# KudanLimited/cuda-bundle-adjustment

Measured on AMD Instinct MI355X. Metric: ba_edge_iterations_per_sec, higher is better.
Workload: dtype f64

## Files before the change

### cuda-bundle-adjustment_amd/csrc/host/c_api.cpp

```cpp
#include <cmath>
#include <cstring>
#include <deque>
#include <memory>
#include <unordered_map>

#include "../../../include/cugo_hip.h"
#include "../../include/cuda_graph_optimisation.h"
#include "../../include/icp_types.h"
#include "../kernels/kernels.h"
#include "chol_solver.h"
#include "edge_layout.h"
#include "engine.h"
#include "hip_util.h"
#include "rccl_comm.h"
#include "schur_plan.h"

using namespace cugo_host;

namespace
{
template <typename F>
int guarded(F&& f)
{
    try
// ... 83 lines not shown
        CUGO_HIP(hipMemcpyAsync(d, h, bytes, hipMemcpyHostToDevice, ctx->stream));
        CUGO_HIP(hipStreamSynchronize(ctx->stream));
    });
}
int cugo_memcpy_d2h(cugo_ctx* ctx, void* h, const void* d, size_t bytes)
{
    return guarded([&] {
        CUGO_HIP(hipMemcpyAsync(h, d, bytes, hipMemcpyDeviceToHost, ctx->stream));
        CUGO_HIP(hipStreamSynchronize(ctx->stream));
    });
}
int cugo_memset(cugo_ctx* ctx, void* d, int value, size_t bytes)
{
    return guarded([&] { CUGO_HIP(hipMemsetAsync(d, value, bytes, ctx->stream)); });
}

int cugo_compute_active_errors(cugo_ctx* ctx, const cugo_edges* ev, const double* d_poses,
                               const double* d_lms, cugo_robust rk, double* d_chi)
{
    return guarded([&] {
        cugo_k::launch_errors(ctx->stream, *ev, d_poses, d_lms, rk, scratch_for(ctx, ev), d_chi);
        CUGO_HIP(hipGetLastError());
    });
}

int cugo_construct_quadratic_form(cugo_ctx* ctx, const cugo_edges* ev, const double* d_poses,
                                  const double* d_lms, cugo_robust rk, double* d_Hpp, double* d_bp,
                                  double* d_Hll, double* d_bl, void* d_Hpl, double* d_chi)
{
    return guarded([&] {
        cugo_k::launch_build(ctx->stream, *ev, d_poses, d_lms, rk, d_Hpp, d_bp, d_Hll, d_bl, d_Hpl,
                             scratch_for(ctx, ev), d_chi);
        CUGO_HIP(hipGetLastError());
    });
}

}

namespace
{
void check_icp_kind(cugo_ctx* ctx, const char* what, int n, int P, const int32_t* d_pose, const int32_t* d_ptr,
                    const double* d_p, const double* d_geo, const double* d_omega, int n_omega, int rk, double delta)
{
    const std::string in = std::string(" (") + what + ")";
    if (n < 0)
        throw std::runtime_error("cugo_icp: negative edge count" + in);
    if (!d_ptr)
        throw std::runtime_error("cugo_icp: no pose_ptr" + in);
    if (rk < CUGO_RK_NONE || rk > CUGO_RK_HUBER || (rk != CUGO_RK_NONE && !(delta > 0.0 && std::isfinite(delta))))
        throw std::runtime_error("cugo_icp: unknown robust kernel or bad delta" + in);
    if (n > 0 && (!d_pose || !d_p || !d_geo || !d_omega || (n_omega != 1 && n_omega != n)))
        throw std::runtime_error("cugo_icp: missing arrays" + in);
    std::vector<int32_t> ptr(P + 1);
    CUGO_HIP(hipMemcpyAsync(ptr.data(), d_ptr, sizeof(int32_t) * (P + 1), hipMemcpyDeviceToHost, ctx->stream));
    CUGO_HIP(hipStreamSynchronize(ctx->stream));
    if (ptr[0] != 0 || ptr[P] != n)
        throw std::runtime_error("cugo_icp: pose_ptr does not span the edges" + in);
    for (int p = 0; p < P; p++)
        if (ptr[p + 1] < ptr[p])
            throw std::runtime_error("cugo_icp: pose_ptr not ascending" + in);
}

void check_icp(cugo_ctx* ctx, const cugo_icp_edges* ev, cugo_k::ReduceScratch rs)
{
    check_icp_kind(ctx, "plane", ev->n_plane, ev->n_poses_total, ev->d_plane_pose, ev->d_plane_pose_ptr, ev->d_plane_p,
                   ev->d_plane_nd, ev->d_plane_omega, ev->n_plane_omega, ev->rk_plane, ev->delta_plane);
    check_icp_kind(ctx, "line", ev->n_line, ev->n_poses_total, ev->d_line_pose, ev->d_line_pose_ptr, ev->d_line_p,
                   ev->d_line_au, ev->d_line_omega, ev->n_line_omega, ev->rk_line, ev->delta_line);
    if (cugo_k::icp_check_indices(ctx->stream, *ev, rs))
        throw std::runtime_error("cugo_icp: edges not sorted by pose, or a pose index disagrees with pose_ptr");
}

void check_icp_counts(const cugo_icp_edges* ev)
{
    if (!ev || ev->n_poses_total < 0 || ev->n_poses_free < 0 || ev->n_poses_free > ev->n_poses_total ||
        ev->n_plane < 0 || ev->n_line < 0)
        throw std::runtime_error("cugo_icp: bad pose or edge counts");
}

cugo_k::ReduceScratch icp_scratch_for(cugo_ctx* ctx, const cugo_icp_edges* ev)
{
    const size_t need = cugo_k::icp_scratch_doubles(*ev);
    if (ctx->scratch.size() < need)
    {
        CUGO_HIP(hipStreamSynchronize(ctx->stream));
        ctx->scratch.resize(need);
    }
    return {ctx->scratch.data(), ctx->scratch.size()};
}
}

extern "C" {

int cugo_icp_compute_errors(cugo_ctx* ctx, const cugo_icp_edges* ev, const double* d_poses, double* d_chi,
                            double* d_edge_chi)
{
    return guarded([&] {
        check_icp_counts(ev);
        const cugo_k::ReduceScratch rs = icp_scratch_for(ctx, ev);
        check_icp(ctx, ev, rs);
        cugo_k::launch_icp_errors(ctx->stream, *ev, d_poses, rs, d_chi, false, d_edge_chi);
        CUGO_HIP(hipGetLastError());
    });
}

int cugo_icp_construct_quadratic_form(cugo_ctx* ctx, const cugo_icp_edges* ev, const double* d_poses, double* d_Hpp,
                                      double* d_bp, double* d_chi)
{
    return guarded([&] {
        check_icp_counts(ev);
        const cugo_k::ReduceScratch rs = icp_scratch_for(ctx, ev);
        check_icp(ctx, ev, rs);
        cugo_k::launch_icp_build(ctx->stream, *ev, d_poses, d_Hpp, d_bp, rs, d_chi, false);
        CUGO_HIP(hipGetLastError());
    });
}

int cugo_max_diagonal(cugo_ctx* ctx, const double* d_Hpp, int nP, const double* d_Hll, int nL,
                      double* d_out)
{
    return guarded([&] {
        cugo_k::launch_max_diagonal(ctx->stream, d_Hpp, nP, d_Hll, nL, scratch_for(ctx, nullptr),
                                    d_out);
        CUGO_HIP(hipGetLastError());
    });
}

int cugo_compute_schur(cugo_ctx* ctx, const cugo_edges* ev, const cugo_hsc_struct* hs, double lambda,
                       int damp_hsc_diag, const double* d_Hpp, const double* d_bp,
                       const double* d_Hll, const double* d_bl, const void* d_Hpl,
                       double* d_invHll, void* d_T, double* d_bsc, double* d_Hsc)
{
    return guarded([&] {
        if (!d_T && !hs->d_grp_ptr)
            throw std::runtime_error("cugo_compute_schur: d_T may only be NULL with a landmark-major plan "
                                     "(cugo_hsc_plan_create); the gather kernels read T from memory");
        cugo_k::SchurRows form;
        form.mfma = ctx->opt.hsc_mfma, form.xcd = ctx->opt.hsc_xcd;
        cugo_k::launch_schur(ctx->stream, *ev, *hs, lambda, damp_hsc_diag, d_Hpp, d_bp, d_Hll, d_bl,
                             d_Hpl, d_invHll, d_T, d_bsc, d_Hsc, false, form);
        CUGO_HIP(hipGetLastError());
    });
}

int cugo_backsubst_update(cugo_ctx* ctx, const cugo_edges* ev, double lambda,
                          const double* d_invHll, const double* d_bl, const double* d_bp,
                          const void* d_Hpl, const double* d_xp, double* d_xl,
                          const double* d_poses_in, const double* d_lms_in, double* d_poses_out,
                          double* d_lms_out, double* d_scale)
{
    return guarded([&] {
        cugo_k::launch_backsubst_update(ctx->stream, *ev, lambda, lambda, d_invHll, d_bl, d_bp, d_Hpl,
                                        d_xp, d_xl, d_poses_in, d_lms_in, d_poses_out, d_lms_out,
                                        scratch_for(ctx, ev), d_scale);
        CUGO_HIP(hipGetLastError());
    });
}

int cugo_chol_create(cugo_ctx* ctx, cugo_chol** out)
{
    return guarded([&] {
        auto* s = new cugo_chol;
        s->ctx = ctx;
        *out = s;
    });
}
void cugo_chol_destroy(cugo_chol* s)
{
    if (s && s->ctx)
        (void)hipStreamSynchronize(s->ctx->stream);
    delete s;
}
int cugo_chol_analyze(cugo_chol* s, int n, const int32_t* rowptr, const int32_t* colind)
{
    return guarded([&] { s->analyze(n, rowptr, colind); });
}
int cugo_chol_factor_solve(cugo_chol* s, const double* d_Hsc, double lambda, const double* d_bsc,
                           double* d_x, int32_t* d_fail)
{
    return guarded([&] {
        if (!s->analyzed || !s->ctx)
            throw std::runtime_error("cugo_chol_factor_solve needs an analysed solver with a device context");
        s->factor_solve(d_Hsc, lambda, d_bsc, d_x, d_fail);
    });
}
int cugo_chol_selected_inverse(cugo_chol* s, double* d_sigma)
{
    bool ok = true;
    const int rc = guarded([&] {
        if (!s || !s->ctx || !s->analyzed || !s->factored)
            throw std::runtime_error("cugo_chol_selected_inverse needs a factorisation (cugo_chol_factor_solve) since the "
                                     "last analyze()");
        if (s->own_subtrees())
            throw std::runtime_error("cugo_chol_selected_inverse: not available when the solver factors rank-owned "
                                     "subtrees");
        ok = s->selected_inverse(d_sigma);
    });
    if (rc != CUGO_OK)
        return rc;
    if (!ok)
    {
        set_last_error("cugo_chol_selected_inverse: the factorisation hit a zero pivot");
        return CUGO_ERR_NUMERIC;
    }
    return CUGO_OK;
}
#ifdef CUGO_DEBUG_HOOKS
int cugo_debug_pin_reference(void)
{
    return guarded([&] { cugo_debug_pin_reference_solver(); });
}
int cugo_debug_dump_call(int which, int call, const char* path)
{
    return guarded([&] {
        cugo_chol* s = cugo_debug_solver(which);
        if (!s)
            throw std::runtime_error("cugo_debug_dump_call: no solver has run with CUGO_DEBUG_KEEP");
        s->dump_slot(call, path);
    });
}
int cugo_debug_plan_array(int which, const char* name, const int32_t** out)
{
    cugo_chol* s = cugo_debug_solver(which);
    if (!s)
        return -1;
    return cugo_chol_plan_array(s, name, out);
}
int cugo_debug_dump(const char* dir, int* n_calls)
{
    return guarded([&] {
        const int n = cugo_debug_dump_last_solver(dir);
        if (n_calls)
            *n_calls = n;
    });
}
#endif
int cugo_chol_stats(const cugo_chol* s, double* nnzL, double* flops, int* n_super, int* n_stages,
                    double* front_bytes)
{
    if (nnzL)
        *nnzL = s->plan.nnzL;
    if (flops)
        *flops = s->plan.flops;
    if (n_super)
        *n_super = s->plan.n_super;
    if (n_stages)
        *n_stages = s->plan.n_stages;
    if (front_bytes)
        *front_bytes = 8.0 * (double)s->plan.front_doubles;
    return CUGO_OK;
}
int cugo_chol_plan_sizes(const cugo_chol* s, int* n, int* n_super, int* n_rows_total)
{
    *n = s->plan.n;
    *n_super = s->plan.n_super;
    *n_rows_total = (int)s->plan.rows.size();
    return CUGO_OK;
}
int cugo_chol_plan_get(const cugo_chol* s, int32_t* perm, int32_t* super_ptr, int32_t* rows_ptr,
                       int32_t* rows, int32_t* parent)
{
    const CholPlan& P = s->plan;
    std::memcpy(perm, P.perm.data(), sizeof(int32_t) * P.perm.size());
    std::memcpy(super_ptr, P.super_ptr.data(), sizeof(int32_t) * P.super_ptr.size());
    std::memcpy(rows_ptr, P.rows_ptr.data(), sizeof(int32_t) * P.rows_ptr.size());
    std::memcpy(rows, P.rows.data(), sizeof(int32_t) * P.rows.size());
    std::memcpy(parent, P.sparent.data(), sizeof(int32_t) * P.sparent.size());
    return CUGO_OK;
}

int cugo_chol_plan_array(cugo_chol* s, const char* name, const int32_t** out)
{
    const CholPlan& P = s->plan;
    const std::string n(name);
    const std::vector<int32_t>* v = nullptr;
#define CUGO_PLAN_FIELD(f) \
    if (n == #f)           \
    v = &P.f
    CUGO_PLAN_FIELD(perm);
    CUGO_PLAN_FIELD(super_ptr);
    CUGO_PLAN_FIELD(rows_ptr);
    CUGO_PLAN_FIELD(rows);
    CUGO_PLAN_FIELD(sparent);
    CUGO_PLAN_FIELD(child_ptr);
    CUGO_PLAN_FIELD(child);
    CUGO_PLAN_FIELD(rel_ptr);
    CUGO_PLAN_FIELD(rel);
    CUGO_PLAN_FIELD(ncb);
    CUGO_PLAN_FIELD(nb);
    CUGO_PLAN_FIELD(col0);
    CUGO_PLAN_FIELD(col_front);
    CUGO_PLAN_FIELD(stage_task_ptr);
    CUGO_PLAN_FIELD(task_ptr);
    CUGO_PLAN_FIELD(task_fronts);
    CUGO_PLAN_FIELD(blk_front);
    CUGO_PLAN_FIELD(blk_row);
    CUGO_PLAN_FIELD(blk_col);
    CUGO_PLAN_FIELD(alias_of);
    CUGO_PLAN_FIELD(asm_map);
    CUGO_PLAN_FIELD(wl);
    CUGO_PLAN_FIELD(bc_front);
    CUGO_PLAN_FIELD(bc_seg_ptr);
    CUGO_PLAN_FIELD(bc_seg);
#undef CUGO_PLAN_FIELD
    if (n == "asm_info")
    {
        s->asm_info.assign(1, P.asm0);
        s->asm_info.push_back(P.nasm);
        for (int64_t o : P.asm_off)
            s->asm_info.push_back((int32_t)o);
        v = &s->asm_info;
    }
    if (n == "blk_trans")
        v = &s->trans32;
    if (n == "ea1")
        v = &s->ea1;
    if (!v)
    {
        set_last_error("cugo_chol_plan_array: unknown array " + n);
        return CUGO_ERR_INVALID;
    }
    *out = v->data();
    return (int)v->size();
}

int cugo_chol_plan_array64(cugo_chol* s, const char* name, const int64_t** out)
{
    const CholPlan& P = s->plan;
    const std::string n(name);
    const std::vector<int64_t>* v = n == "off" ? &P.off : n == "ldf" ? &P.ldf : n == "woff" ? &P.woff
                                  : n == "l21off" ? &P.l21off : nullptr;
    if (!v)
    {
        set_last_error("cugo_chol_plan_array64: unknown array " + n);
        return CUGO_ERR_INVALID;
    }
    *out = v->data();
    return (int)v->size();
}

int cugo_shard_range(int n_landmarks_total, const int32_t* edges_per_landmark, int rank, int world,
                     int* l0, int* l1)
{
    return guarded([&] {
        if (world < 1 || rank < 0 || rank >= world)
            throw std::runtime_error("cugo_shard_range: bad rank/world");
        std::vector<int32_t> cnt(n_landmarks_total + 1, 0);
        for (int l = 0; l < n_landmarks_total; l++)
            cnt[l + 1] = cnt[l] + edges_per_landmark[l];
        shard_range(cnt, rank, world, *l0, *l1);
    });
}

struct cugo_graph
{
    cugo::GraphOptimisationOptions options;
    std::unique_ptr<cugo::CudaGraphOptimisationImpl> opt;
    cugo::PoseVertexSet poses{false};
    cugo::LandmarkVertexSet lms{true};
    cugo::MonoEdgeSet mono;
    cugo::StereoEdgeSet stereo;
    cugo::PlaneEdgeSet plane;
    cugo::LineEdgeSet line;
    std::deque<cugo::PlaneEdge> plane_store;
    std::deque<cugo::LineEdge> line_store;
    std::deque<cugo::PoseVertex> pose_store;
    std::deque<cugo::LandmarkVertex> lm_store;
    std::deque<cugo::MonoEdge> mono_store;
    std::deque<cugo::StereoEdge> stereo_store;
    bool attached = false;
    void attach()
    {
        if (attached)
            return;
        opt->addVertexSet(&poses);
        opt->addVertexSet(&lms);
        opt->addEdgeSet(&mono);
        opt->addEdgeSet(&stereo);
        opt->addEdgeSet(&plane);
        opt->addEdgeSet(&line);
        attached = true;
    }
};

int cugo_graph_create(int per_edge_information, int per_edge_camera, cugo_graph** out)
{
    return guarded([&] {
        auto g = std::make_unique<cugo_graph>();
        g->options.perEdgeInformation = per_edge_information != 0;
        g->options.perEdgeCamera = per_edge_camera != 0;
        g->opt = std::make_unique<cugo::CudaGraphOptimisationImpl>(g->options);
        *out = g.release();
    });
}
struct cugo_hsc_plan
{
    cugo_host::SchurPlanDevice dev;
};
int cugo_hsc_plan_create(cugo_ctx* ctx, int n_edges, int n_poses_free, const int32_t* h_pose, const int32_t* h_lm,
                         const uint8_t* h_flags, const int32_t* h_rowptr, const int32_t* h_colind,
                         cugo_hsc_struct* hs, cugo_hsc_plan** out)
{
    int rc = guarded([&] {
        if (!ctx || !hs || !out)
            throw std::runtime_error("cugo_hsc_plan_create: null argument");
        *out = nullptr;
        cugo_host::SchurPlanDevice::clear(*hs);
        cugo_host::SchurPlanHost h;
        cugo_host::build_schur_plan(n_edges, n_poses_free, h_pose, h_lm, h_flags, h_rowptr, h_colind, h);
        if (!h.usable)
            throw std::invalid_argument("cugo_hsc_plan_create: a landmark's active edges straddle two 256-slot groups");
        auto p = std::make_unique<cugo_hsc_plan>();
        p->dev.upload(h, ctx->stream);
        p->dev.fill(*hs);
        *out = p.release();
    });
    return rc;
}
void cugo_hsc_plan_destroy(cugo_hsc_plan* plan) { delete plan; }

int cugo_graph_create_plan_only(int per_edge_information, int per_edge_camera, cugo_graph** out)
{
    return guarded([&] {
        auto g = std::make_unique<cugo_graph>();
        g->options.perEdgeInformation = per_edge_information != 0;
        g->options.perEdgeCamera = per_edge_camera != 0;
        g->options.planOnly = true;
        g->opt = std::make_unique<cugo::CudaGraphOptimisationImpl>(g->options);
        *out = g.release();
    });
}
void cugo_graph_destroy(cugo_graph* g) { delete g; }

int cugo_graph_add_poses(cugo_graph* g, int n, const int32_t* ids, const double* qt, const uint8_t* fixed)
{
    return guarded([&] {
        for (int i = 0; i < n; i++)
        {
            g->pose_store.emplace_back(ids[i], cugo::Se3D(qt + 7 * (size_t)i, qt + 7 * (size_t)i + 4),
                                       fixed && fixed[i]);
            g->poses.addVertex(&g->pose_store.back());
        }
    });
}
int cugo_graph_add_landmarks(cugo_graph* g, int n, const int32_t* ids, const double* xyz,
                             const uint8_t* fixed)
{
    return guarded([&] {
        for (int i = 0; i < n; i++)
        {
            g->lm_store.emplace_back(ids[i], cugo::Vec3d(xyz + 3 * (size_t)i), fixed && fixed[i]);
            g->lms.addVertex(&g->lm_store.back());
        }
    });
}
int cugo_graph_add_edges(cugo_graph* g, int dim, int n, const int32_t* pose_ids, const int32_t* lm_ids,
                         const double* meas, const double* info, const double* cam5)
{
    return guarded([&] {
        if (dim != 2 && dim != 3)
            throw std::runtime_error("cugo_graph_add_edges: dim must be 2 or 3");
        for (int i = 0; i < n; i++)
        {
            cugo::PoseVertex* vp = g->poses.getVertex(pose_ids[i]);
            cugo::LandmarkVertex* vl = g->lms.getVertex(lm_ids[i]);
            cugo::Camera cam;
            if (cam5)
                cam = cugo::Camera(cam5[5 * (size_t)i], cam5[5 * (size_t)i + 1], cam5[5 * (size_t)i + 2],
                                   cam5[5 * (size_t)i + 3], cam5[5 * (size_t)i + 4]);
            if (dim == 2)
            {
                g->mono_store.emplace_back();
                cugo::MonoEdge& e = g->mono_store.back();
                e.setVertex(vp, 0), e.setVertex(vl, 1);
                e.setMeasurement(cugo::Vec2d(meas + 2 * (size_t)i));
                e.setInformation(info ? info[i] : 0.0);
                if (cam5)
                    e.setCamera(cam);
                g->mono.addEdge(&e);
            }
            else
            {
                g->stereo_store.emplace_back();
                cugo::StereoEdge& e = g->stereo_store.back();
                e.setVertex(vp, 0), e.setVertex(vl, 1);
                e.setMeasurement(cugo::Vec3d(meas + 3 * (size_t)i));
                e.setInformation(info ? info[i] : 0.0);
                if (cam5)
                    e.setCamera(cam);
                g->stereo.addEdge(&e);
            }
        }
    });
}
static cugo::PoseVertex* icp_pose(cugo_graph* g, int32_t id)
{
    try
    {
        return g->poses.getVertex(id);
    }
    catch (const std::out_of_range&)
    {
        throw std::invalid_argument("cugo_graph_add_*_edges: unknown pose id " + std::to_string(id));
    }
}
int cugo_graph_add_plane_edges(cugo_graph* g, int n, const int32_t* pose_ids, const double* pointP,
                               const double* normal, const double* origin_distance, const double* info)
{
    return guarded([&] {
        if (n < 0 || (n > 0 && (!pose_ids || !pointP || !normal || !origin_distance)))
            throw std::invalid_argument("cugo_graph_add_plane_edges: missing arrays");
        for (int i = 0; i < n; i++)
            (void)icp_pose(g, pose_ids[i]);
        for (int i = 0; i < n; i++)
        {
            g->plane_store.emplace_back();
            cugo::PlaneEdge& e = g->plane_store.back();
            e.setVertex(icp_pose(g, pose_ids[i]), 0);
            e.setMeasurement(cugo::PointToPlaneMatch<double>(cugo::Vec3d(normal + 3 * (size_t)i), origin_distance[i],
                                                             cugo::Vec3d(pointP + 3 * (size_t)i)));
            e.setInformation(info ? info[i] : 0.0);
            g->plane.addEdge(&e);
        }
    });
}
int cugo_graph_add_line_edges(cugo_graph* g, int n, const int32_t* pose_ids, const double* pointP, const double* a,
                              const double* b, const double* info)
{
    return guarded([&] {
        if (n < 0 || (n > 0 && (!pose_ids || !pointP || !a || !b)))
            throw std::invalid_argument("cugo_graph_add_line_edges: missing arrays");
        for (int i = 0; i < n; i++)
            (void)icp_pose(g, pose_ids[i]);
        for (int i = 0; i < n; i++)
        {
            g->line_store.emplace_back();
            cugo::LineEdge& e = g->line_store.back();
            e.setVertex(icp_pose(g, pose_ids[i]), 0);
            cugo::PointToLineMatch<double> mz(cugo::Vec3d(a + 3 * (size_t)i), cugo::Vec3d(b + 3 * (size_t)i));
            mz.pointP = cugo::Vec3d(pointP + 3 * (size_t)i);
            e.setMeasurement(mz);
            e.setInformation(info ? info[i] : 0.0);
            g->line.addEdge(&e);
        }
    });
}
static cugo::BaseEdgeSet* icp_set(cugo_graph* g, int kind)
{
    if (kind == CUGO_ICP_PLANE)
        return &g->plane;
    if (kind == CUGO_ICP_LINE)
        return &g->line;
    throw std::invalid_argument("cugo: kind must be CUGO_ICP_PLANE (0) or CUGO_ICP_LINE (1)");
}
int cugo_graph_set_icp_information(cugo_graph* g, int kind, double info)
{
    return guarded([&] { icp_set(g, kind)->setInformation(info); });
}
int cugo_graph_set_icp_robust_kernel(cugo_graph* g, int kind, int type, double delta)
{
    return guarded([&] {
        const cugo::RobustKernelType t = type == CUGO_RK_CAUCHY  ? cugo::RobustKernelType::Cauchy
                                         : type == CUGO_RK_TUKEY ? cugo::RobustKernelType::Tukey
                                         : type == CUGO_RK_HUBER ? cugo::RobustKernelType::Huber
                                                                 : cugo::RobustKernelType::None;
        icp_set(g, kind)->setRobustKernel(t, delta);
    });
}
int cugo_graph_set_icp_outlier_threshold(cugo_graph* g, int kind, double threshold)
{
    return guarded([&] {
        if (kind == CUGO_ICP_PLANE)
            g->plane.setOutlierThreshold(threshold);
        else if (kind == CUGO_ICP_LINE)
            g->line.setOutlierThreshold(threshold);
        else
            icp_set(g, kind);
    });
}
int cugo_graph_n_icp_edges(cugo_graph* g, int kind)
{
    return kind == CUGO_ICP_PLANE || kind == CUGO_ICP_LINE ? g->opt->nIcpEdges(kind) : -1;
}
int cugo_graph_set_camera(cugo_graph* g, int dim, const double* c)
{
    const cugo::Camera cam(c[0], c[1], c[2], c[3], c[4]);
    if (dim == 3)
        g->stereo.setCamera(cam);
    else
        g->mono.setCamera(cam);
    return CUGO_OK;
}
int cugo_graph_set_information(cugo_graph* g, int dim, double info)
{
    if (dim == 3)
        g->stereo.setInformation(info);
    else
        g->mono.setInformation(info);
    return CUGO_OK;
}
int cugo_graph_set_robust_kernel(cugo_graph* g, int dim, int type, double delta)
{
    const cugo::RobustKernelType t = type == CUGO_RK_CAUCHY  ? cugo::RobustKernelType::Cauchy
                                     : type == CUGO_RK_TUKEY ? cugo::RobustKernelType::Tukey
                                     : type == CUGO_RK_HUBER ? cugo::RobustKernelType::Huber
                                                             : cugo::RobustKernelType::None;
// ... 282 lines not shown
```

### cuda-bundle-adjustment_amd/csrc/host/chol_solver.cpp

```cpp
#include "chol_solver.h"

#include <cstdio>
#include <cstdlib>
#include <cstring>
#include <string>

using namespace cugo_host;

void cugo_chol::pack()
{
    const CholPlan& P = plan;
    pack32.clear(), pack64.clear();
    auto put32 = [this](const std::vector<int32_t>& v) {
        const size_t o = pack32.size();
        pack32.insert(pack32.end(), v.begin(), v.end());
        pack32.resize((pack32.size() + 3) & ~size_t(3));
        return o;
    };
    auto put64 = [this](const std::vector<int64_t>& v) {
        const size_t o = pack64.size();
        pack64.insert(pack64.end(), v.begin(), v.end());
        pack64.resize((pack64.size() + 1) & ~size_t(1));
        return o;
    };
    const size_t o_ncb = put32(P.ncb), o_nb = put32(P.nb), o_col0 = put32(P.col0);
    const size_t o_alias = put32(P.alias_of), o_bwnp = put32(P.bw_np), o_lanp = put32(P.la_np);
    const size_t o_rows_ptr = put32(P.rows_ptr), o_rows = put32(P.rows);
    const size_t o_child_ptr = put32(P.child_ptr), o_child = put32(P.child);
    const size_t o_rel_ptr = put32(P.rel_ptr), o_rel = put32(P.rel);
    const size_t o_task_ptr = put32(P.task_ptr), o_task_fronts = put32(P.task_fronts);
    const size_t o_blk_front = put32(P.blk_front), o_blk_row = put32(P.blk_row), o_blk_col = put32(P.blk_col);
    const size_t o_perm = put32(P.perm), o_col_front = put32(P.col_front), o_wl = put32(P.wl);
    const size_t ntask = P.task_ptr.empty() ? 0 : P.task_ptr.size() - 1;
    constexpr int R = cugo_k::EA1_REC;
    std::vector<int32_t> ea1_ptr(P.n_super + 1, 0);
    ea1.clear();
    for (int f = 0; f < P.n_super; f++)
    {
        if (P.alias_of[f] < 0)
            for (int k = P.child_ptr[f]; k < P.child_ptr[f + 1]; k++)
            {
                const int c = P.child[k];
                const int64_t ncs_c = 6 * (int64_t)P.ncb[c], ldc = P.ldf[c];
                const int64_t q[2] = {P.off[c] + ncs_c * ldc + ncs_c, ldc};
                int32_t r[R] = {c, P.nb[c] - P.ncb[c], P.la_np[c], P.rel_ptr[c]};
                std::memcpy(r + 4, q, sizeof q);
                uint32_t mask = 0;
                for (int b = 0; b < P.la_np[c]; b++)
                {
                    const int pr = P.rel[P.rel_ptr[c] + b];
                    if (pr < 0 || pr >= 32 || pr >= P.ncb[f])
                        throw std::runtime_error("cugo: a child's leading row lies outside its parent's pivot block");
                    mask |= 1u << pr;
                }
                r[8] = (int32_t)mask;
                ea1.insert(ea1.end(), r, r + R);
            }
        ea1_ptr[f + 1] = (int32_t)(ea1.size() / R);
    }
    const size_t n_ea1 = ea1.size();
    ea1.resize(n_ea1 + R, 0);
    const size_t o_ea1 = put32(ea1);
    ea1.resize(n_ea1);
    std::vector<int32_t> tmeta(cugo_k::TMETA * ntask, 0);
    for (size_t t = 0; t < ntask; t++)
    {
        int32_t* m = tmeta.data() + cugo_k::TMETA * t;
        const int f = P.task_fronts[P.task_ptr[t]];
        m[0] = P.task_ptr[t + 1] - P.task_ptr[t], m[1] = f, m[2] = P.ncb[f], m[3] = P.nb[f], m[4] = P.col0[f];
        m[5] = P.bw_np[f], m[6] = P.rows_ptr[f];
        m[7] = (P.alias_of[f] < 0 && P.child_ptr[f + 1] > P.child_ptr[f]) ? 1 : 0;
        m[16] = ea1_ptr[f], m[17] = ea1_ptr[f + 1];
        for (int q = 0; q < 16; q++)
        {
            const int nrows = P.rows_ptr[f + 1] - P.rows_ptr[f];
            m[20 + q] = nrows > 0 ? P.rows[P.rows_ptr[f] + std::min(q, nrows - 1)] : 0;
        }
        const int64_t q[4] = {P.off[f], P.ldf[f], P.woff[f], P.l21off[f]};
        std::memcpy(m + 8, q, sizeof q);
    }
    const size_t o_tmeta = put32(tmeta);
    std::vector<int32_t> fat(16 * (P.wl.size() / 3), 0);
    for (size_t i = 0; i < P.wl.size() / 3; i++)
    {
        int32_t* m = fat.data() + 16 * i;
        const int f = P.wl[3 * i];
        m[0] = f, m[1] = P.wl[3 * i + 1], m[2] = P.wl[3 * i + 2];
        if (f < 0 || f >= P.n_super)
            continue;
        m[3] = 6 * P.ncb[f], m[4] = 6 * (P.nb[f] - P.ncb[f]);
        m[5] = P.bw_np[f], m[6] = P.col0[f], m[7] = P.rows_ptr[f];
        const int64_t q[4] = {P.off[f], P.ldf[f], P.woff[f], P.l21off[f]};
        std::memcpy(m + 8, q, sizeof q);
        if ((int)i >= P.asm0 && (int)i < P.asm0 + P.nasm)
        {
            const int64_t nb = P.nb[f], mo = P.asm_off[f];
            m[5] = (int32_t)nb;
            std::memcpy(m + 6, &mo, sizeof mo);
            bool any = false;
            for (int64_t cb = m[1]; cb < m[2]; cb++)
            {
                any = any || P.asm_map[mo + cb] >= 0;
                const int64_t c0 = mo + nb + cb * nb - cb * (cb - 1) / 2;
                for (int64_t k = 0; k < nb - cb && !any; k++)
                    any = P.asm_map[c0 + k] >= 0;
            }
            m[4] = any ? 1 : 0;
        }
    }
    const size_t o_fat = put32(fat);
    std::vector<int32_t> bc_rec(cugo_k::BC_REC * P.bc_front.size(), 0), bc_seg(4 * (P.bc_seg.size() / 3) + 4, 0);
    for (size_t t = 0; t < P.bc_front.size(); t++)
    {
        int32_t* m = bc_rec.data() + cugo_k::BC_REC * t;
        const int f = P.bc_front[t];
        m[0] = f, m[1] = P.ncb[f], m[2] = P.nb[f], m[3] = P.col0[f], m[4] = P.rows_ptr[f];
        m[5] = P.bc_seg_ptr[f], m[6] = P.bc_seg_ptr[f + 1] - P.bc_seg_ptr[f];
        const int64_t q[4] = {P.woff[f], P.l21off[f], P.off[f], P.ldf[f]};
        std::memcpy(m + 8, q, sizeof q);
    }
    for (size_t k = 0; k < P.bc_seg.size() / 3; k++)
        std::memcpy(bc_seg.data() + 4 * k, P.bc_seg.data() + 3 * k, 3 * sizeof(int32_t));
    const size_t o_bc_rec = put32(bc_rec), o_bc_seg = put32(bc_seg);
    const size_t o_asm_map = put32(P.asm_map);
    const size_t o_trans = pack32.size();
    pack32.resize(o_trans + (P.blk_trans.size() + 3) / 4 + 4, 0);
    if (!P.blk_trans.empty())
        std::memcpy(pack32.data() + o_trans, P.blk_trans.data(), P.blk_trans.size());
    const size_t o_asm_off = put64(P.asm_off);
    const size_t o_off = put64(P.off), o_woff = put64(P.woff), o_l21off = put64(P.l21off), o_ldf = put64(P.ldf);
    po = {o_ncb, o_nb, o_col0, o_alias, o_bwnp, o_lanp, o_rows_ptr, o_rows, o_child_ptr, o_child, o_rel_ptr, o_rel,
          o_task_ptr, o_task_fronts, o_blk_front, o_blk_row, o_blk_col, o_perm, o_col_front, o_wl, o_ea1, o_tmeta,
          o_fat, o_asm_map, o_trans, o_asm_off, o_off, o_woff, o_l21off, o_ldf, o_bc_rec, o_bc_seg};
}

void cugo_chol::upload(hipStream_t s)
{
    const CholPlan& P = plan;
    const size_t o_ncb = po[0], o_nb = po[1], o_col0 = po[2], o_alias = po[3], o_bwnp = po[4], o_lanp = po[5];
    const size_t o_rows_ptr = po[6], o_rows = po[7], o_child_ptr = po[8], o_child = po[9], o_rel_ptr = po[10];
    const size_t o_rel = po[11], o_task_ptr = po[12], o_task_fronts = po[13], o_blk_front = po[14], o_blk_row = po[15];
    const size_t o_blk_col = po[16], o_perm = po[17], o_col_front = po[18], o_wl = po[19], o_ea1 = po[20];
    const size_t o_tmeta = po[21], o_fat = po[22], o_asm_map = po[23], o_trans = po[24], o_asm_off = po[25];
    const size_t o_off = po[26], o_woff = po[27], o_l21off = po[28], o_ldf = po[29];
    const size_t o_bc_rec = po[30], o_bc_seg = po[31];
    d_pack32.upload(pack32, s), d_pack64.upload(pack64, s);
    d_fronts.resize((size_t)P.front_doubles + 16);
    d_fronts.zero(s);
    d_xnew.resize((size_t)6 * P.n + 16);
    d_junk.resize(64 * 1024);
    d_winv.resize((size_t)P.winv_doubles + 16);
    d_l21.resize((size_t)P.l21_doubles + 16);
    bw_chain = opt.bw_chain && !opt.lookahead && !P.has_subtree_stage && !P.bc_front.empty();
    if (bw_chain)
    {
        d_bc_state.resize((size_t)cugo_k::BC_DONE + P.n_super);
        d_bc_state.zero(s);
        h_bc_error.resize(1);
        h_bc_error[0] = 0;
        bc_base = 0, bc_epoch = 0;
    }
    CUGO_HIP(hipStreamSynchronize(s));

    cugo_k::CholPlanDev& D = dev;
    D.n_fronts = P.n_super;
    const int32_t* b32 = d_pack32.data();
    const int64_t* b64 = d_pack64.data();
    D.ncb = b32 + o_ncb, D.nb = b32 + o_nb, D.off = b64 + o_off, D.col0 = b32 + o_col0;
    D.rows_ptr = b32 + o_rows_ptr, D.rows = b32 + o_rows;
    D.child_ptr = b32 + o_child_ptr, D.child = b32 + o_child;
    D.rel_ptr = b32 + o_rel_ptr, D.rel = b32 + o_rel;
    D.n_stages = P.n_stages;
    D.task_ptr = b32 + o_task_ptr, D.task_fronts = b32 + o_task_fronts, D.tmeta = b32 + o_tmeta;
    D.n_hsc_blocks = (int)P.blk_front.size();
    D.blk_front = b32 + o_blk_front, D.blk_row = b32 + o_blk_row;
    D.blk_col = b32 + o_blk_col, D.blk_trans = reinterpret_cast<const uint8_t*>(b32 + o_trans);
    D.n = P.n, D.perm = b32 + o_perm, D.col_front = b32 + o_col_front;
    D.junk = d_junk.data();
    D.woff = b64 + o_woff, D.winv = d_winv.data(), D.nc_max = P.nc_max;
    D.ea_lds = opt.ea_lds, D.panel16 = opt.panel16, D.ea_direct = opt.ea_direct;
#ifdef CUGO_DEBUG_HOOKS
    {
        const char* ka = std::getenv("CUGO_KERNEL_ACQUIRE");
        D.kernel_acquire = ka ? std::atoi(ka) & 7 : 0;
        const char* ed = std::getenv("CUGO_DEBUG_DELAY");
        D.dbg_delay = ed ? std::atoi(ed) : 0;
        const char* ez = std::getenv("CUGO_DEBUG_ZERO_LDS");
        D.zero_lds = ez ? std::atoi(ez) : 0, D.lds_doubles = 0;
        D.dbg_skip_wg = -1;
    }
#endif
    D.l21off = b64 + o_l21off, D.l21 = d_l21.data();
    D.ldf = b64 + o_ldf, D.alias_of = b32 + o_alias, D.bw_np = b32 + o_bwnp, D.la_np = b32 + o_lanp;
    d_wl_ptr = b32 + o_wl;
    D.wl_base = d_wl_ptr, D.fat = b32 + o_fat, D.ea1 = b32 + o_ea1;
    D.asm_map = b32 + o_asm_map, D.asm_off = b64 + o_asm_off;
    D.bc_rec = b32 + o_bc_rec, D.bc_seg = b32 + o_bc_seg;
    asm_fronts = opt.asm_fronts;
    lds_factor = cugo_k::chol_lds_factor_bytes(P.nc_max);
    lds_backward = cugo_k::chol_lds_backward_bytes(P.nc_max, P.ld_max);
}

void cugo_chol::analyze(int n, const int32_t* rowptr, const int32_t* colind)
{
    analyze_host(n, rowptr, colind);
    if (ctx)
        upload(ctx->stream);
}

void cugo_chol::analyze_host(int n, const int32_t* rowptr, const int32_t* colind)
{
    CholOptions copt = CholOptions::from_env();
    const bool own_forced = opt.own_subtrees == 1;
    if ((world > 1 || own_forced) && bcast && opt.own_subtrees != 0)
        copt.rank = rank, copt.world = world, copt.owned = true;
    chol_analyze(n, rowptr, colind, copt, plan);
    if (copt.owned && !own_forced && plan.flops < 1e9 * opt.own_min_gflop)
    {
        copt.rank = 0, copt.world = 1, copt.owned = false;
        chol_analyze(n, rowptr, colind, copt, plan);
    }
    lookahead = opt.lookahead;
    factored = false, si_ready = false, last_fail = nullptr;
    trans32.assign(plan.blk_trans.begin(), plan.blk_trans.end());
    pack();
    if (plan.nc_max > cugo_k::chol_max_pivot_cols() ||
        cugo_k::chol_lds_factor_bytes(plan.nc_max) > 160 * 1024 ||
        cugo_k::chol_lds_backward_bytes(plan.nc_max, plan.ld_max) > 160 * 1024)
        throw std::runtime_error("cugo: a front exceeds the LDS budget (nc=" +
                                 std::to_string(plan.nc_max) + ", ld=" + std::to_string(plan.ld_max) + ")");
    analyzed = true;
}

#ifdef CUGO_DEBUG_HOOKS
static cugo_chol* g_last_kept = nullptr;
static cugo_chol* g_ref_kept = nullptr;
cugo_chol::~cugo_chol()
{
    if (g_last_kept == this)
        g_last_kept = nullptr;
    if (g_ref_kept == this)
        g_ref_kept = nullptr;
}
void cugo_chol::dump_kept(const char* dir)
{
    CUGO_HIP(hipStreamSynchronize(ctx->stream));
    const size_t nf = (size_t)plan.front_doubles, nw = (size_t)plan.winv_doubles, nl = (size_t)plan.l21_doubles,
                 nx = (size_t)6 * plan.n;
    for (size_t c = 0; c < keep.size(); c++)
    {
        std::vector<double> h(nf + nw + nl + 2 * nx);
        if (keep[c]->size() < h.size())
            continue;
        CUGO_HIP(hipMemcpy(h.data(), keep[c]->data(), h.size() * sizeof(double), hipMemcpyDeviceToHost));
        const std::string path = std::string(dir) + "/call" + std::to_string(c) + ".bin";
        std::FILE* f = std::fopen(path.c_str(), "wb");
        if (!f)
            throw std::runtime_error("cugo_debug_dump: cannot write " + path);
        const int64_t hdr[8] = {(int64_t)nf, (int64_t)nw, (int64_t)nl, (int64_t)nx, (int64_t)nx, 0, 0, 0};
        std::fwrite(hdr, sizeof hdr, 1, f);
        std::fwrite(h.data(), sizeof(double), h.size(), f);
        std::fclose(f);
    }
}
int cugo_debug_dump_last_solver(const char* dir)
{
    if (!g_last_kept)
        return 0;
    g_last_kept->dump_kept(dir);
    return (int)g_last_kept->keep.size();
}
cugo_chol* cugo_debug_solver(int which) { return which ? g_ref_kept : g_last_kept; }
void cugo_debug_pin_reference_solver() { g_ref_kept = g_last_kept; }
void cugo_chol::dump_slot(int call, const char* path)
{
    CUGO_HIP(hipStreamSynchronize(ctx->stream));
    const size_t nf = (size_t)plan.front_doubles, nw = (size_t)plan.winv_doubles, nl = (size_t)plan.l21_doubles,
                 nx = (size_t)6 * plan.n, total = nf + nw + nl + 2 * nx;
    if (call < 0 || call >= (int)keep.size() || keep[call]->size() < total)
        throw std::runtime_error("cugo_debug_dump_call: no such slot");
    std::vector<double> h(total);
    CUGO_HIP(hipMemcpy(h.data(), keep[call]->data(), total * sizeof(double), hipMemcpyDeviceToHost));
    std::FILE* f = std::fopen(path, "wb");
    if (!f)
        throw std::runtime_error(std::string("cugo_debug_dump_call: cannot write ") + path);
    const int64_t hdr[8] = {(int64_t)nf, (int64_t)nw, (int64_t)nl, (int64_t)nx, (int64_t)nx, 0, 0, 0};
    std::fwrite(hdr, sizeof hdr, 1, f);
    std::fwrite(h.data(), sizeof(double), h.size(), f);
    std::fclose(f);
}

struct cugo_chol_hooks
{
    cugo_chol& c;
    hipStream_t s;
    bool skip_on = false;
    double* stale_line = nullptr;
    int stale_stage = -1, stale_kind = -1;
    bool hash_levels, gap, keep_on;
    explicit cugo_chol_hooks(cugo_chol& solver) : c(solver), s(solver.ctx->stream)
    {
        const char* hl = std::getenv("CUGO_DEBUG_HASH_LEVELS");
        hash_levels = !(hl && hl[0] == '0');
        gap = std::getenv("CUGO_DEBUG_GAP") != nullptr;
        keep_on = std::getenv("CUGO_DEBUG_KEEP") != nullptr;
        const cugo_host::CholPlan& plan = c.plan;
        const char* sk = std::getenv("CUGO_DEBUG_SKIP");
        const char* dump = c.dbg_calls == 0 ? std::getenv("CUGO_DEBUG_SKIP_DUMP") : nullptr;
        int cc = -1, l = -1, w = -1;
        if (sk && std::sscanf(sk, "%d:%d:%d", &cc, &l, &w) == 3 && cc == c.dbg_calls)
            cugo_k::chol_dbg_skip_begin(l, w, dump), skip_on = true;
        else if (dump)
            cugo_k::chol_dbg_skip_begin(-1, -1, dump), skip_on = true;
        c.dbg_calls++;
        const char* sl = std::getenv("CUGO_DEBUG_STALE");
        int kind = -1;
        long line = -1;
        if (sl && std::sscanf(sl, "%d:%d:%ld", &cc, &kind, &line) == 3 && cc == c.dbg_calls - 1 && line >= 0)
        {
            std::vector<int> stage_of(plan.n_super, 0);
            for (int st = 0; st < plan.n_stages; st++)
                for (int t = plan.stage_task_ptr[st]; t < plan.stage_task_ptr[st + 1]; t++)
                    for (int fi = plan.task_ptr[t]; fi < plan.task_ptr[t + 1]; fi++)
                        stage_of[plan.task_fronts[fi]] = st;
            const int64_t e = 16 * (int64_t)line;
            if (kind == 0 && e + 16 <= plan.winv_doubles)
            {
                int f = 0;
                for (int k = 0; k < plan.n_super; k++)
                    if (plan.woff[k] <= e && plan.woff[k] >= plan.woff[f])
                        f = k;
                stale_line = c.d_winv.data() + e, stale_stage = stage_of[f], stale_kind = 0;
            }
            else if (kind == 1 && e + 16 <= 6LL * plan.n)
                stale_line = c.d_xnew.data() + e, stale_stage = stage_of[plan.col_front[e / 6]], stale_kind = 1;
            if (stale_line)
            {
                c.dbg_scratch.resize(16);
                CUGO_HIP(hipMemcpyAsync(c.dbg_scratch.data(), stale_line, 16 * sizeof(double), hipMemcpyDeviceToDevice, s));
            }
        }
    }
    ~cugo_chol_hooks()
    {
        if (skip_on)
            cugo_k::chol_dbg_skip_end();
    }
    void hash(int slot, const double* ptr, size_t n)
    {
        if (c.dbg_hash && slot < 64)
            cugo_k::launch_hash_words(s, ptr, n, c.dbg_hash + slot);
    }
    void after_level(int st)
    {
        if (hash_levels && st < 24)
        {
            hash(16 + st, c.d_winv.data(), (size_t)c.plan.winv_doubles);
            hash(40 + st, c.d_fronts.data(), (size_t)c.plan.front_doubles);
        }
        if (gap)
            cugo_k::launch_nop(s);
    }
    double* stale_for_potrf(int st) const { return stale_kind == 0 && stale_stage == st ? stale_line : nullptr; }
    void after_two_phase(int st)
    {
        if (stale_kind == 0 && stale_stage == st)
            cugo_k::launch_swap16(s, stale_line, c.dbg_scratch.data());
    }
    void after_backward(int st)
    {
        if (stale_kind == 1 && (st == stale_stage || st == stale_stage - 1))
            cugo_k::launch_swap16(s, stale_line, c.dbg_scratch.data());
    }
    void keep_arrays(double* d_x)
    {
        if (!keep_on || c.dbg_calls > 16)
            return;
        const cugo_host::CholPlan& plan = c.plan;
        const size_t nf = (size_t)plan.front_doubles, nw = (size_t)plan.winv_doubles, nl = (size_t)plan.l21_doubles,
                     nx = (size_t)6 * plan.n;
        while (c.keep.size() < (size_t)c.dbg_calls)
            c.keep.emplace_back(new cugo_host::DevBuf<double>());
        auto& k = *c.keep[c.dbg_calls - 1];
        k.resize(nf + nw + nl + 2 * nx + 8);
        double* dst = k.data();
        const std::pair<const double*, size_t> parts[] = {{c.d_fronts.data(), nf}, {c.d_winv.data(), nw}, {c.d_l21.data(), nl},
                                                          {c.d_xnew.data(), nx}, {d_x, nx}};
        for (const auto& pr : parts)
        {
            if (pr.second)
                CUGO_HIP(hipMemcpyAsync(dst, pr.first, pr.second * sizeof(double), hipMemcpyDeviceToDevice, s));
            dst += pr.second;
        }
        g_last_kept = &c;
    }
};
#define CUGO_HOOK(expr) expr
#else
cugo_chol::~cugo_chol() {}
#define CUGO_HOOK(expr) ((void)0)
#endif

void cugo_chol::factor_solve(const double* d_Hsc, double lambda, const double* d_bsc, double* d_x,
                             int32_t* d_fail)
{
    hipStream_t s = ctx->stream;
    check_chain_error();
    factored = true, last_fail = d_fail;
#ifdef CUGO_DEBUG_HOOKS
    cugo_chol_hooks hooks(*this);
#endif
#ifdef CUGO_STAMPS
    static const bool dbg = std::getenv("CUGO_DEBUG_STAMPS") != nullptr;
    static long long* d_stamps = nullptr;
    if (dbg && !d_stamps)
    {
        CUGO_HIP(hipMalloc(reinterpret_cast<void**>(&d_stamps), 64 * sizeof(long long)));
        CUGO_HIP(hipMemset(d_stamps, 0, 64 * sizeof(long long)));
        cugo_k::set_debug_stamps(d_stamps);
    }
#endif
    cugo_k::launch_chol_assemble(s, dev, d_fronts.data(), (size_t)plan.front_doubles, d_Hsc, lambda, d_bsc, d_fail,
                                 d_wl_ptr + 3L * plan.clr0, plan.nclr, asm_fronts ? d_wl_ptr + 3L * plan.asm0 : nullptr,
                                 plan.nasm);
    CUGO_HOOK(hooks.hash(11, d_fronts.data(), (size_t)plan.front_doubles));
    int pend0 = 0, npend = 0, pend_tile = 64;
    for (int st = 0; st < plan.n_stages; st++)
    {
        const int t0 = plan.stage_task_ptr[st], t1 = plan.stage_task_ptr[st + 1];
        if (plan.has_subtree_stage && st == 0)
            cugo_k::launch_chol_subtree_stage(s, dev, d_fronts.data(), t0, t1 - t0, lds_factor, d_fail);
        else if (lookahead)
        {
            cugo_k::launch_chol_potrf_la(s, dev, d_fronts.data(), t0, t1 - t0, d_wl_ptr + 3L * pend0, npend,
                                         pend_tile, d_fail);
            cugo_k::launch_chol_lead(s, dev, d_fronts.data(), d_wl_ptr + 3L * plan.lead_ptr[st],
                                     plan.lead_ptr[st + 1] - plan.lead_ptr[st], d_wl_ptr + 3L * plan.ea_ptr[st],
                                     plan.ea_ptr[st + 1] - plan.ea_ptr[st], d_wl_ptr + 3L * plan.eab_ptr[st],
                                     plan.eab_ptr[st + 1] - plan.eab_ptr[st]);
            pend0 = plan.sb_ptr[st], npend = plan.sb_ptr[st + 1] - plan.sb_ptr[st];
            pend_tile = plan.stage_tile[st] ? plan.stage_tile[st] : 64;
        }
        else
        {
            double* stale = nullptr;
            double* stale_scratch = nullptr;
            CUGO_HOOK((stale = hooks.stale_for_potrf(st), stale_scratch = dbg_scratch.data()));
            cugo_k::launch_chol_upper_stage(
                s, dev, d_fronts.data(), t0, t1 - t0, d_wl_ptr, plan.ea_ptr[st],
                plan.ea_ptr[st + 1] - plan.ea_ptr[st], plan.eab_ptr[st],
                plan.eab_ptr[st + 1] - plan.eab_ptr[st], plan.syrk_ptr[st],
                plan.syrk_ptr[st + 1] - plan.syrk_ptr[st], plan.stage_tile[st], lds_factor, d_fail, stale, stale_scratch);
            if (plan.stage_tile[st] == 0)
            {
                cugo_k::launch_chol_two_phase(s, dev, d_fronts.data(), d_wl_ptr + 3L * plan.trsm_ptr[st],
                                              plan.trsm_ptr[st + 1] - plan.trsm_ptr[st],
                                              d_wl_ptr + 3L * plan.syrk_ptr[st],
                                              plan.syrk_ptr[st + 1] - plan.syrk_ptr[st]);
                CUGO_HOOK(hooks.after_two_phase(st));
            }
        }
        CUGO_HOOK(hooks.after_level(st));
        bool grouped = false;
        for (size_t k = 0; k < plan.xu_front.size(); k++)
            if (plan.xu_stage[k] == st)
            {
                if (!grouped && bcast_group)
                    bcast_group(true), grouped = true;
                const int f = plan.xu_front[k];
                const int64_t ld = plan.ldf[f], c0 = 6LL * plan.ncb[f], c1 = 6LL * plan.nb[f];
                if (c1 > c0)
                    bcast(d_fronts.data() + plan.off[f] + c0 * ld + c0, (size_t)((c1 - 1 - c0) * ld + c1 + 1 - c0),
                          plan.xu_owner[k]);
            }
        if (grouped)
            bcast_group(false);
    }
    if (npend > 0)
        cugo_k::launch_chol_potrf_la(s, dev, d_fronts.data(), 0, 0, d_wl_ptr + 3L * pend0, npend, pend_tile, d_fail);
    CUGO_HOOK(hooks.hash(12, d_winv.data(), (size_t)plan.winv_doubles));
    CUGO_HOOK(hooks.hash(13, d_l21.data(), (size_t)plan.l21_doubles));
    CUGO_HOOK(hooks.hash(14, d_fronts.data(), (size_t)plan.front_doubles));
    if (bw_chain)
    {
        const int nf = (int)plan.bc_front.size();
        if (++bc_epoch == 0)
            bc_epoch = 1;
        cugo_k::launch_chol_backward_chain(s, dev, d_fronts.data(), nf, d_xnew.data(), d_x, d_bc_state.data(), bc_base,
                                           bc_epoch, d_fail, h_bc_error.data());
        bc_base += (uint32_t)nf;
#ifdef CUGO_STAMPS
        if (dbg)
        {
            static int chain_calls = 0;
            static long long* d_cs = nullptr;
            if (++chain_calls == 4)
            {
                CUGO_HIP(hipMalloc(reinterpret_cast<void**>(&d_cs), 3 * sizeof(long long) * (size_t)nf));
                CUGO_HIP(hipMemset(d_cs, 0, 3 * sizeof(long long) * (size_t)nf));
                cugo_k::set_chain_stamps(d_cs);
            }
            if (chain_calls == 5)
            {
                std::vector<long long> h(3 * (size_t)nf);
                std::vector<int> ticket(plan.n_super, -1);
                for (int t = 0; t < nf; t++)
                    ticket[plan.bc_front[t]] = t;
                CUGO_HIP(hipStreamSynchronize(s));
                CUGO_HIP(hipMemcpy(h.data(), d_cs, h.size() * sizeof(long long), hipMemcpyDeviceToHost));
                cugo_k::set_chain_stamps(nullptr);
                long long first = h[0], last = 0;
                for (int t = 0; t < nf; t++)
                    first = std::min(first, h[3 * t]), last = std::max(last, h[3 * t + 2]);
                std::printf("chain stamps: %d fronts, first start to last done %lld ticks (10 ns)\n", nf, last - first);
                for (int f = plan.bc_front[nf - 1]; f >= 0; f = plan.sparent[f])
                {
                    const int t = ticket[f], pa = plan.sparent[f];
                    std::printf("  front %d ticket %d ncb %d rows %d: start +%lld", f, t, plan.ncb[f], plan.nb[f] - plan.ncb[f],
                                h[3 * t] - first);
                    if (pa >= 0)
                        std::printf(" wait %lld work %lld", h[3 * t + 1] - h[3 * ticket[pa] + 2], h[3 * t + 2] - h[3 * t + 1]);
                    std::printf(" done +%lld\n", h[3 * t + 2] - first);
                }
            }
        }
#endif
    }
    for (int st = plan.n_stages - 1; st >= 0 && !bw_chain; st--)
    {
        const int t0 = plan.stage_task_ptr[st], t1 = plan.stage_task_ptr[st + 1];
        cugo_k::launch_chol_backward_stage(s, dev, d_fronts.data(), t0, t1 - t0, lds_backward, d_xnew.data(),
                                           d_x, d_wl_ptr + 3L * plan.bwg_ptr[st],
                                           plan.bwg_ptr[st + 1] - plan.bwg_ptr[st]);
        CUGO_HOOK(hooks.after_backward(st));
#ifdef CUGO_STAMPS
        if (dbg && st == plan.n_stages - 1)
        {
            CUGO_HIP(hipStreamSynchronize(s));
            CUGO_HIP(hipMemcpy(d_stamps + 48, d_stamps + 24, 8 * sizeof(long long), hipMemcpyDeviceToDevice));
        }
#endif
    }
    CUGO_HOOK(hooks.hash(15, d_xnew.data(), (size_t)6 * plan.n));
    if (!plan.xx_lo.empty())
    {
        if (bcast_group)
            bcast_group(true);
        for (size_t k = 0; k < plan.xx_lo.size(); k++)
            bcast(d_xnew.data() + 6LL * plan.xx_lo[k], (size_t)(6LL * (plan.xx_hi[k] - plan.xx_lo[k])), plan.xx_owner[k]);
        if (bcast_group)
            bcast_group(false);
        cugo_k::launch_chol_unpermute(s, dev, d_xnew.data(), d_x);
    }
    CUGO_HIP(hipGetLastError());
    CUGO_HOOK(hooks.keep_arrays(d_x));
#ifdef CUGO_STAMPS
    if (dbg)
    {
        long long h[64];
        CUGO_HIP(hipStreamSynchronize(s));
        CUGO_HIP(hipMemcpy(h, d_stamps, sizeof h, hipMemcpyDeviceToHost));
        static int calls = 0;
        if (++calls == 5)
            for (int k = 0; k < 7; k++)
            {
                std::printf("stamps kernel %d (nc=%lld):", k, h[k * 8 + 6]);
                for (int i = 1; i < 8; i++)
                    if (i != 6 && h[k * 8 + i])
                        std::printf(" [%d] +%lld", i, h[k * 8 + i] - h[k * 8]);
                std::printf("  (cycles since kernel start; last launch of the kernel)\n");
            }
    }
#endif
}

void cugo_chol::check_chain_error()
{
    if (bw_chain && h_bc_error.data() && *static_cast<volatile uint32_t*>(h_bc_error.data()) != 0)
        throw std::runtime_error("cugo: the backward substitution gave up waiting for a front (k_backward_chain)");
}

bool cugo_chol::selected_inverse(double* d_sigma)
{
    hipStream_t s = ctx->stream;
    int32_t h_fail = 0;
    CUGO_HIP(hipMemcpyAsync(&h_fail, last_fail, sizeof h_fail, hipMemcpyDeviceToHost, s));
    CUGO_HIP(hipStreamSynchronize(s));
    check_chain_error();
    if (h_fail)
        return false;
    const CholPlan& P = plan;
    if (!si_ready)
    {
        std::vector<int64_t> sinfo(4 * (size_t)P.n_super + 4, 0);
        for (int f = 0; f < P.n_super; f++)
        {
            const int pa = P.sparent[f];
            if (pa < 0)
                continue;
            sinfo[4 * f] = P.off[pa], sinfo[4 * f + 1] = P.ldf[pa], sinfo[4 * f + 2] = P.rel_ptr[f];
            sinfo[4 * f + 3] = P.alias_of[pa] == f ? 0 : 1;
        }
        const int tile = cugo_k::selinv_row_tile();
        std::vector<int32_t> items;
        si_ptr.assign(P.n_stages + 1, 0);
        for (int st = 0; st < P.n_stages; st++)
        {
            si_ptr[st] = (int32_t)(items.size() / 2);
            if (!(P.has_subtree_stage && st == 0))
                for (int t = P.stage_task_ptr[st]; t < P.stage_task_ptr[st + 1]; t++)
                    for (int fi = P.task_ptr[t]; fi < P.task_ptr[t + 1]; fi++)
                    {
                        const int f = P.task_fronts[fi];
                        for (int r0 = 0; r0 < 6 * (P.nb[f] - P.ncb[f]); r0 += tile)
                            items.push_back(f), items.push_back(r0);
                    }
        }
        si_ptr[P.n_stages] = (int32_t)(items.size() / 2);
        items.resize(items.size() + 2, 0);
        d_sinfo.upload(sinfo, s);
        d_sitems.upload(items, s);
        d_sig.resize((size_t)P.front_doubles + 16);
        d_sig.zero(s);
        CUGO_HIP(hipStreamSynchronize(s));
        si_ready = true;
    }
    for (int st = P.n_stages - 1; st >= 0; st--)
    {
        const int t0 = P.stage_task_ptr[st], t1 = P.stage_task_ptr[st + 1];
        if (P.has_subtree_stage && st == 0)
            cugo_k::launch_selinv_subtree(s, dev, d_fronts.data(), d_sig.data(), d_sinfo.data(), t0, t1 - t0);
        else
        {
            cugo_k::launch_selinv_rows(s, dev, d_fronts.data(), d_sig.data(), d_sinfo.data(),
                                       d_sitems.data() + 2L * si_ptr[st], si_ptr[st + 1] - si_ptr[st]);
            cugo_k::launch_selinv_jj(s, dev, d_fronts.data(), d_sig.data(), t0, t1 - t0);
        }
    }
    cugo_k::launch_selinv_gather(s, dev, d_sig.data(), d_sigma);
    CUGO_HIP(hipGetLastError());
    return true;
}
```

### cuda-bundle-adjustment_amd/csrc/host/chol_solver.h

```cpp
#pragma once
#include "../kernels/kernels.h"
#include "chol_symbolic.h"
#include "hip_util.h"
#include "options.h"

#include <array>
#include <functional>
#include <memory>

struct cugo_chol
{
    cugo_ctx* ctx = nullptr;
    bool analyzed = false;
    cugo_host::Options opt = cugo_host::Options::from_env();
    cugo_host::CholPlan plan;
    std::vector<int32_t> trans32;
    std::vector<int32_t> asm_info;
    std::vector<int32_t> ea1;
    cugo_k::CholPlanDev dev{};
    size_t lds_factor = 0, lds_backward = 0;
    bool lookahead = false;
    bool asm_fronts = true;

    std::vector<int32_t> pack32;
    std::vector<int64_t> pack64;
    std::array<size_t, 32> po{};
    cugo_host::DevBuf<int32_t> d_pack32;
    cugo_host::DevBuf<int64_t> d_pack64;
    const int32_t* d_wl_ptr = nullptr;
    cugo_host::DevBuf<double> d_fronts, d_xnew, d_junk, d_winv, d_l21;
    bool bw_chain = false;
    cugo_host::DevBuf<uint32_t> d_bc_state;
    cugo_host::PinnedBuf<uint32_t> h_bc_error;
    uint32_t bc_base = 0, bc_epoch = 0;
    void check_chain_error();

    int rank = 0, world = 1;
    std::function<void(double*, size_t, int)> bcast;
    std::function<void(bool)> bcast_group;
    ~cugo_chol();
#ifdef CUGO_DEBUG_HOOKS
    unsigned long long* dbg_hash = nullptr;
    int dbg_calls = 0;
    std::vector<std::unique_ptr<cugo_host::DevBuf<double>>> keep;
    cugo_host::DevBuf<double> dbg_scratch;
    void dump_kept(const char* dir);
    void dump_slot(int call, const char* path);
#endif
    bool own_subtrees() const { return bcast && plan.owned; }

    const int32_t* last_fail = nullptr;
    bool factored = false;
    bool si_ready = false;
    cugo_host::DevBuf<double> d_sig;
    cugo_host::DevBuf<int64_t> d_sinfo;
    cugo_host::DevBuf<int32_t> d_sitems;
    std::vector<int32_t> si_ptr;
    bool selected_inverse(double* d_sigma);

    void analyze(int n, const int32_t* rowptr, const int32_t* colind);
    void analyze_host(int n, const int32_t* rowptr, const int32_t* colind);
    void pack();
    void upload(hipStream_t s);
    void factor_solve(const double* d_Hsc, double lambda, const double* d_bsc, double* d_x,
                      int32_t* d_fail);
};

#ifdef CUGO_DEBUG_HOOKS
int cugo_debug_dump_last_solver(const char* dir);
cugo_chol* cugo_debug_solver(int which);
void cugo_debug_pin_reference_solver();
#endif
```

### cuda-bundle-adjustment_amd/csrc/host/chol_symbolic.cpp

```cpp
#include "chol_symbolic.h"

#include <algorithm>
#include <atomic>
#include <chrono>
#include <cstdio>
#include <cstdlib>
#include <functional>
#include <numeric>
#include <stdexcept>
#include <thread>
#include <tuple>

namespace cugo_host
{

CholOptions CholOptions::from_env()
{
    CholOptions o;
    if (const char* s = std::getenv("CUGO_ND_LEAF"))
        o.nd_leaf = std::max(1, std::atoi(s));
    if (const char* s = std::getenv("CUGO_MAX_SUPER_COLS"))
        o.max_super_cols = std::max(1, std::atoi(s));
    if (const char* s = std::getenv("CUGO_ZERO_FRAC"))
        o.zero_frac = std::atof(s);
// ... 1176 lines not shown
        P.nc_max = std::max(P.nc_max, 6 * P.ncb[s]);
    P.ea_ptr.assign(1, 0), P.eab_ptr.assign(1, 0), P.syrk_ptr.assign(1, 0), P.bwg_ptr.assign(1, 0);
    P.lead_ptr.assign(1, 0), P.sb_ptr.assign(1, 0);
    P.bw_np.assign(ns, -1);
    P.la_np.assign(ns, 0);
    for (int c = 0; c < ns; c++)
        if (P.sparent[c] >= 0)
        {
            const int nbr = P.nb[c] - P.ncb[c], ncbp = P.ncb[P.sparent[c]];
            int np = 0;
            while (np < nbr && P.rel[P.rel_ptr[c] + np] < ncbp)
                np++;
            P.la_np[c] = np;
        }
    std::vector<int32_t> lead, sb;
    P.l21off.assign(ns, -1);
    P.l21_doubles = 0;
    std::vector<int32_t> ea, eab, sy, bwg, tr;
    std::vector<int> sy_front_ntiles;
    P.trsm_ptr.assign(1, 0);
    P.stage_tile.assign(P.n_stages, 64);
    for (int st = 0; st < P.n_stages; st++)
    {
        const bool subtree = P.has_subtree_stage && st == 0;
        int TS = 64;
        bool two_phase = false;
        if (!subtree)
        {
            long n64 = 0;
            for (int t = P.stage_task_ptr[st]; t < P.stage_task_ptr[st + 1]; t++)
            {
                const int f = P.task_fronts[P.task_ptr[t]];
                const long nti = (6 * (P.nb[f] - P.ncb[f]) + 1 + 63) / 64;
                n64 += nti * (nti + 1) / 2;
            }
            if (n64 <= opt.tile32_max_tiles)
                TS = 32;
            P.stage_tile[st] = TS;
            two_phase = opt.two_phase_min_tiles > 0 && n64 > opt.two_phase_min_tiles;
            if (two_phase)
                P.stage_tile[st] = 0;
        }
        if (!subtree)
            for (int t = P.stage_task_ptr[st]; t < P.stage_task_ptr[st + 1]; t++)
            {
                const int f = P.task_fronts[P.task_ptr[t]];
                const int nb = P.nb[f], ncb = P.ncb[f];
                {
                    const double nc = 6.0 * ncb, nr = 6.0 * (nb - ncb);
                    P.up_potrf_flops += nc * nc * nc / 3.0;
                    P.up_trsm_flops += nc * nc * (nr + 1);
                    P.up_syrk_flops += 2.0 * nc * (nr * (nr + 1) / 2 + nr);
                    for (int k = P.child_ptr[f]; k < P.child_ptr[f + 1] && P.alias_of[f] < 0; k++)
                    {
                        const double cr = 6.0 * (P.nb[P.child[k]] - P.ncb[P.child[k]]);
                        P.up_ea_bytes += 24.0 * (cr * (cr + 1) / 2 + cr);
                    }
                }
                if (P.child_ptr[f + 1] > P.child_ptr[f] && P.alias_of[f] < 0)
                {
                    const int chunks = (6 * nb + 1 + 63) / 64;
                    const int cols = std::max(1, std::min(8, 16 / chunks));
                    for (int c0 = 0; c0 < ncb; c0 += cols)
                    {
                        ea.push_back(f), ea.push_back(c0), ea.push_back(std::min(ncb, c0 + cols));
                    }
                    for (int c0 = ncb; c0 < nb; c0 += cols)
                    {
                        eab.push_back(f), eab.push_back(c0), eab.push_back(std::min(nb, c0 + cols));
                    }
                }
                const int nrs = 6 * (nb - ncb), nbelow = nrs + 1;
                const int nti = (nbelow + TS - 1) / TS, ntj = (nrs + TS - 1) / TS;
                const size_t sy_front0 = sy.size();
                if (two_phase)
                {
                    int ntl = 0;
                    for (int tj = 0; tj < ntj; tj++)
                        ntl += nti - tj;
                    for (int t = 0; t < ntl; t++)
                    {
                        sy.push_back(f), sy.push_back(t), sy.push_back(ntj);
                    }
                    for (int r0 = 0; r0 < nbelow; r0 += 64)
                    {
                        tr.push_back(f), tr.push_back(r0), tr.push_back(std::min(64, nbelow - r0));
                    }
                }
                else
                {
                    for (int tj = 0; tj < ntj; tj++)
                        for (int ti = tj; ti < nti; ti++)
                        {
                            sy.push_back(f), sy.push_back(ti), sy.push_back(tj);
                        }
                    for (int ti = ntj; ti < nti; ti++)
                    {
                        sy.push_back(f), sy.push_back(ti), sy.push_back(-1);
                    }
                }
                sy_front_ntiles.push_back(std::max(1, (int)((sy.size() - sy_front0) / 3)));
                const int q = 6 * P.la_np[f];
                if (q > 0)
                {
                    lead.push_back(f), lead.push_back(0), lead.push_back(0);
                }
                for (int tj = 0; tj < ntj; tj++)
                    for (int ti = tj; ti < nti; ti++)
                        if (TS * (ti + 1) > q)
                        {
                            sb.push_back(f), sb.push_back(ti), sb.push_back(tj);
                        }
                for (int ti = ntj; ti < nti; ti++)
                {
                    sb.push_back(f), sb.push_back(ti), sb.push_back(-1);
                }
                P.l21off[f] = P.l21_doubles;
                P.l21_doubles += (int64_t)6 * ncb * nbelow;
                for (int k = P.child_ptr[f]; k < P.child_ptr[f + 1]; k++)
                {
                    const int c = P.child[k];
                    if (lower[c] || !mine(c))
                        continue;
                    const int nbr = P.nb[c] - P.ncb[c];
                    int npb = 0;
                    while (npb < nbr && P.rel[P.rel_ptr[c] + npb] < ncb)
                        npb++;
                    if (nbr - npb >= 8)
                    {
                        P.bw_np[c] = npb;
                        for (int j0 = 0; j0 < 6 * P.ncb[c]; j0 += 16)
                        {
                            bwg.push_back(c), bwg.push_back(j0), bwg.push_back(0);
                        }
                    }
                }
            }
        if (!subtree && opt.xcd_affinity && !sy_front_ntiles.empty())
        {
            const int nf = (int)sy_front_ntiles.size();
            int total = 0;
            for (int n : sy_front_ntiles)
                total += n;
            if (total > 8)
            {
                std::vector<int> byn(nf);
                for (int i = 0; i < nf; i++)
                    byn[i] = i;
                std::stable_sort(byn.begin(), byn.end(), [&](int a, int b) { return sy_front_ntiles[a] > sy_front_ntiles[b]; });
                std::vector<int> load(8, 0);
                std::vector<int> group_of(P.n_super, 0);
                for (int i : byn)
                {
                    const int g = (int)(std::min_element(load.begin(), load.end()) - load.begin());
                    group_of[P.task_fronts[P.task_ptr[P.stage_task_ptr[st] + i]]] = g;
                    load[g] += sy_front_ntiles[i];
                }
                auto interleave = [&](std::vector<int32_t>& list, size_t first, int phase) {
                    const int n = (int)(list.size() / 3 - first);
                    if (n <= 1)
                        return;
                    std::vector<std::vector<int>> grp(8);
                    for (int k = 0; k < n; k++)
                        grp[group_of[list[3 * (first + k)]]].push_back(k);
                    std::vector<int32_t> out;
                    out.reserve((size_t)n * 3);
                    std::vector<size_t> pos(8, 0);
                    for (int k = 0; k < n; k++)
                    {
                        const int g = (phase + k) & 7;
                        int t;
                        if (pos[g] < grp[g].size())
                            t = grp[g][pos[g]++];
                        else
                        {
                            int best = 0;
                            size_t left = 0;
                            for (int h = 0; h < 8; h++)
                                if (grp[h].size() - pos[h] > left)
                                    left = grp[h].size() - pos[h], best = h;
                            t = grp[best].back();
                            grp[best].pop_back();
                        }
                        out.insert(out.end(), list.begin() + 3 * (first + t), list.begin() + 3 * (first + t) + 3);
                    }
                    std::copy(out.begin(), out.end(), list.begin() + 3 * first);
                };
                interleave(sy, (size_t)P.syrk_ptr.back(), 0);
                interleave(tr, (size_t)P.trsm_ptr.back(), 0);
            }
        }
        sy_front_ntiles.clear();
        P.ea_ptr.push_back((int)ea.size() / 3);
        P.eab_ptr.push_back((int)eab.size() / 3);
        P.syrk_ptr.push_back((int)sy.size() / 3);
        P.trsm_ptr.push_back((int)tr.size() / 3);
        P.bwg_ptr.push_back((int)bwg.size() / 3);
        P.lead_ptr.push_back((int)lead.size() / 3);
        P.sb_ptr.push_back((int)sb.size() / 3);
    }
    P.wl.clear();
    P.wl.insert(P.wl.end(), ea.begin(), ea.end());
    P.wl.insert(P.wl.end(), eab.begin(), eab.end());
    P.wl.insert(P.wl.end(), sy.begin(), sy.end());
    P.wl.insert(P.wl.end(), bwg.begin(), bwg.end());
    for (auto& v : P.eab_ptr)
        v += (int)ea.size() / 3;
    for (auto& v : P.syrk_ptr)
        v += (int)(ea.size() + eab.size()) / 3;
    for (auto& v : P.bwg_ptr)
        v += (int)(ea.size() + eab.size() + sy.size()) / 3;
    for (auto& v : P.trsm_ptr)
        v += (int)P.wl.size() / 3;
    P.wl.insert(P.wl.end(), tr.begin(), tr.end());
    P.clr0 = (int)P.wl.size() / 3;
    P.nclr = 0;
    for (int f = 0; f < ns; f++)
        if (P.alias_of[f] < 0 && mine(f))
            for (int c0 = 0; c0 < 6 * P.nb[f]; c0 += 16)
            {
                P.wl.push_back(f), P.wl.push_back(c0), P.wl.push_back(std::min(6 * P.nb[f], c0 + 16));
                P.nclr++;
            }
    P.asm0 = (int)P.wl.size() / 3;
    P.nasm = 0;
    P.asm_off.assign(ns, -1);
    P.asm_map.clear();
    {
        std::vector<int32_t> root(ns), shift(ns);
        for (int f = 0; f < ns; f++)
        {
            int o = f;
            while (P.alias_of[o] >= 0)
                o = P.alias_of[o];
            const int64_t delta = P.off[f] - P.off[o], ld = P.ldf[o];
            if (P.ldf[f] != ld || delta % (ld + 1) != 0 || (delta / (ld + 1)) % 6 != 0 ||
                delta / (ld + 1) / 6 + P.nb[f] != P.nb[o])
                throw std::runtime_error("cugo: a front stored inside another one is not on its diagonal");
            root[f] = o, shift[f] = (int)(delta / (ld + 1) / 6);
        }
        for (int f = 0; f < ns; f++)
            if (P.alias_of[f] < 0 && mine(f))
            {
                const int64_t nb = P.nb[f];
                P.asm_off[f] = (int64_t)P.asm_map.size();
                P.asm_map.resize(P.asm_map.size() + nb + nb * (nb + 1) / 2, -1);
                for (int cb = 0; cb < nb; cb += 2)
                {
                    P.wl.push_back(f), P.wl.push_back(cb), P.wl.push_back((int)std::min<int64_t>(nb, cb + 2));
                    P.nasm++;
                }
            }
        for (int f = 0; f < ns; f++)
            if (P.asm_off[root[f]] >= 0)
                for (int c = 0; c < P.ncb[f]; c++)
                    P.asm_map[P.asm_off[root[f]] + shift[f] + c] = P.col0[f] + c;
        for (size_t k = 0; k < P.blk_front.size(); k++)
        {
            const int f = P.blk_front[k], o = root[f];
            if (P.asm_off[o] < 0)
                continue;
            const int64_t nb = P.nb[o], rb = P.blk_row[k] + shift[f], cb = P.blk_col[k] + shift[f];
            if (rb < cb || rb >= nb)
                throw std::runtime_error("cugo: an Hsc block outside the lower triangle of its front");
            int32_t& e = P.asm_map[P.asm_off[o] + nb + cb * nb - cb * (cb - 1) / 2 + (rb - cb)];
            if (e != -1)
                throw std::runtime_error("cugo: two Hsc blocks in one front position");
            e = 2 * (int32_t)k + (rb != cb && P.blk_trans[k] ? 1 : 0);
        }
    }
    for (auto& v : P.lead_ptr)
        v += (int)P.wl.size() / 3;
    P.wl.insert(P.wl.end(), lead.begin(), lead.end());
    for (auto& v : P.sb_ptr)
        v += (int)P.wl.size() / 3;
    P.wl.insert(P.wl.end(), sb.begin(), sb.end());
    lap("8 work items");
    P.bc_front.clear(), P.bc_seg.clear();
    P.bc_seg_ptr.assign(ns + 1, 0);
    std::vector<int32_t> ticket(ns, -1);
    for (int st = P.n_stages - 1; st >= 0; st--)
        for (int t = P.stage_task_ptr[st]; t < P.stage_task_ptr[st + 1]; t++)
            for (int fi = P.task_ptr[t + 1] - 1; fi >= P.task_ptr[t]; fi--)
            {
                ticket[P.task_fronts[fi]] = (int32_t)P.bc_front.size();
                P.bc_front.push_back(P.task_fronts[fi]);
            }
    for (int f = 0; f < ns; f++)
    {
        const int r0 = P.rows_ptr[f], r1 = P.rows_ptr[f + 1];
        for (int k = r0; k < r1;)
        {
            const int a = P.col_front[P.rows[k]];
            int e = k + 1;
            while (e < r1 && e - k < 16 && P.col_front[P.rows[e]] == a)
                e++;
            if (ticket[f] >= 0 && !(ticket[a] >= 0 && ticket[a] < ticket[f]))
                throw std::runtime_error("cugo: a boundary row of a front belongs to a front scheduled after it");
            P.bc_seg.push_back(a), P.bc_seg.push_back(k - r0), P.bc_seg.push_back(e - k);
            k = e;
        }
        P.bc_seg_ptr[f + 1] = (int32_t)(P.bc_seg.size() / 3);
    }
    lap("9 backward chain");
}

}
```

### cuda-bundle-adjustment_amd/csrc/host/chol_symbolic.h

```cpp
#pragma once
#include <cstdint>
#include <vector>

namespace cugo_host
{

struct CholOptions
{
    int nd_refine = 1;
    int nd_leaf = 96;
    int max_super_cols = 16;
    double zero_frac = 0.35;
    int target_tasks = 1024;
    bool alias_chains = true;
    int min_subtree_tasks = 1 << 30;
    int max_front_cols = 16;
    int two_phase_min_tiles = 260;
    bool xcd_affinity = true;
    int tile32_max_tiles = 64;
    int rank = 0, world = 1;
    bool owned = false;
    static CholOptions from_env();
};

struct CholPlan
{
    int n = 0;
    std::vector<int32_t> perm, iperm;

    int n_super = 0;
    std::vector<int32_t> super_ptr;
    std::vector<int32_t> rows_ptr, rows;
    std::vector<int32_t> sparent;
    std::vector<int32_t> child_ptr, child;
    std::vector<int32_t> rel_ptr, rel;
    std::vector<int32_t> ncb, nb, col0;
    std::vector<int64_t> off;
    int64_t front_doubles = 0;
    std::vector<int64_t> ldf;
    std::vector<int32_t> alias_of;
    int n_aliased = 0;
    std::vector<int64_t> woff;
    int64_t winv_doubles = 0;
    std::vector<int64_t> l21off;
    int64_t l21_doubles = 0;
    std::vector<int32_t> col_front;

    int n_stages = 0;
    int sum_slots = 0;
    int nd_refined = 0;
    std::vector<int32_t> stage_task_ptr;
    std::vector<int32_t> task_ptr, task_fronts;
    bool has_subtree_stage = false;
    std::vector<int32_t> wl;
    std::vector<int32_t> ea_ptr, eab_ptr, syrk_ptr, bwg_ptr;
    int clr0 = 0, nclr = 0;
    int asm0 = 0, nasm = 0;
    std::vector<int32_t> asm_map;
    std::vector<int64_t> asm_off;
    std::vector<int32_t> la_np;
    std::vector<int32_t> lead_ptr, sb_ptr;
    std::vector<int32_t> stage_tile;
    std::vector<int32_t> trsm_ptr;
    std::vector<int32_t> bw_np;
    std::vector<int32_t> bc_front, bc_seg_ptr, bc_seg;
    int nc_max = 6;

    std::vector<int32_t> owner;
    std::vector<int32_t> xu_front, xu_stage, xu_owner;
    std::vector<int32_t> xx_lo, xx_hi, xx_owner;
    double rank_flops = 0, top_flops = 0;
    bool owned = false;
    int64_t xs_seg = 0, xs_top = 0;
    std::vector<int64_t> xs_off;

    std::vector<int32_t> blk_front, blk_row, blk_col;
    std::vector<uint8_t> blk_trans;

    long ld_max = 1;
    double nnzL = 0;
    double flops = 0;
    double up_potrf_flops = 0, up_trsm_flops = 0, up_syrk_flops = 0, up_ea_bytes = 0, backward_bytes = 0;
};

void chol_analyze(int n, const int32_t* rowptr, const int32_t* colind, const CholOptions& opt,
                  CholPlan& plan);

}
```

### cuda-bundle-adjustment_amd/csrc/host/options.h

```cpp
#pragma once
#include <cstdlib>

namespace cugo_host
{

struct Options
{
    int hsc_mfma = 1;
    bool hsc_xcd = true;
    bool hsc_rows = false, hsc_strip = false, schur_plan = false;
    bool fuse_t = true;
    bool pose_schur = true;
    bool float32 = false;
    bool speculate = true, trial_event = true, trial_poll = true;
    bool trial_from_build = true;
    bool profile = false;
    bool init_timing = false;
    bool structure_reuse = true;
    bool flatten_reuse = true;
    bool async_structure = true;
    bool host_structure = false;
    bool upload_thread = true;
    int own_subtrees = -1;
    double own_min_gflop = 3.0;
    bool lookahead = false;
    bool ea_lds = true, panel16 = true, asm_fronts = true;
    bool ea_direct = true;
    bool bw_chain = true;
    bool reduce_scatter = true;

    static Options from_env()
    {
        Options o;
        auto flag = [](const char* name) { return std::getenv(name) != nullptr; };
        auto off = [](const char* name) {
            const char* e = std::getenv(name);
            return e && e[0] == '0';
        };
        auto on = [](const char* name) {
            const char* e = std::getenv(name);
            return e && e[0] == '1';
        };
        if (const char* e = std::getenv("CUGO_HSC_MFMA"))
            o.hsc_mfma = e[0] == '0' ? 0 : e[0] == '2' ? 2 : 1;
        o.hsc_xcd = !off("CUGO_HSC_XCD");
        o.schur_plan = flag("CUGO_SCHUR_PLAN");
        o.hsc_rows = on("CUGO_HSC_ROWS"), o.hsc_strip = on("CUGO_HSC_STRIP");
        o.fuse_t = !off("CUGO_FUSE_T");
        o.pose_schur = !off("CUGO_POSE_SCHUR");
        o.float32 = on("CUGO_FLOAT32");
        o.speculate = !off("CUGO_SPECULATE"), o.trial_event = !off("CUGO_TRIAL_EVENT"), o.trial_poll = !off("CUGO_TRIAL_POLL");
        o.trial_from_build = !off("CUGO_TRIAL_FROM_BUILD");
        o.profile = flag("CUGO_PROFILE");
        o.init_timing = flag("CUGO_INIT_TIMING");
        o.structure_reuse = !flag("CUGO_NO_STRUCTURE_REUSE");
        o.flatten_reuse = !flag("CUGO_NO_FLATTEN_REUSE");
        o.async_structure = !off("CUGO_ASYNC_STRUCTURE");
        o.host_structure = flag("CUGO_HOST_STRUCTURE");
        o.upload_thread = !off("CUGO_UPLOAD_THREAD");
        if (const char* e = std::getenv("CUGO_OWN_SUBTREES"))
            o.own_subtrees = e[0] == '1' ? 1 : e[0] == '0' ? 0 : -1;
        if (const char* e = std::getenv("CUGO_OWN_MIN_GFLOP"))
            o.own_min_gflop = std::atof(e);
        if (const char* e = std::getenv("CUGO_LOOKAHEAD"))
            o.lookahead = std::atoi(e) != 0;
        o.ea_lds = !off("CUGO_EA_LDS"), o.panel16 = !off("CUGO_PANEL16"), o.asm_fronts = !off("CUGO_ASM_FRONTS");
        o.ea_direct = !off("CUGO_EA_DIRECT");
        o.bw_chain = !off("CUGO_BW_CHAIN");
        o.reduce_scatter = !off("CUGO_REDUCE_SCATTER");
        return o;
    }
};

}
```

### cuda-bundle-adjustment_amd/csrc/kernels/chol_kernels.hip

```cpp
#include <algorithm>
#include <cstdio>

#include "kernels.h"

namespace
{

constexpr int CBS = 256;
constexpr double PIVOT_TOL = 1e-14;
constexpr int TR = 64;
constexpr int NC_MAX = 96;
constexpr int LLD = NC_MAX + 17;
constexpr int PW = 6;

using cugo_k::CholPlanDev;
typedef double double4_t __attribute__((ext_vector_type(4)));

__device__ __forceinline__ void assemble_scatter(const CholPlanDev& p, double* __restrict__ fronts,
                                                 const double* __restrict__ Hsc, double lambda,
                                                 const double* __restrict__ bsc, int32_t* __restrict__ fail, int nblk,
                                                 int bid)
{
    if (bid >= nblk)
    {
// ... 1892 lines not shown
        dev_extend_add(p, fronts, it[0], it[1], it[2], 2);
        kernel_release(p);
        return;
    }
    stamp(0, 0);
    if (DBG_DELAY(p) == 5)
        dbg_sleep();
    if (DBG_DELAY(p) == 29)
        return;
    dbg_fill_lds(p, lds);
    const int32_t* tm = p.tmeta + cugo_k::TMETA * (task0 + blockIdx.x);
    const long* tm64 = reinterpret_cast<const long*>(tm + 8);
    const int f = tm[1];
    const int ncs = 6 * tm[2];
    const long foff = tm64[0], fld = tm64[1], fwoff = tm64[2];
    const int ncp = pad16(ncs);
    double* Ls = lds;
    double* dinv = lds + NC_MAX * LLD;
    double* Vs = dinv + NC_MAX;
    const bool kids = tm[7] != 0;
    if (kids && !p.ea_lds)
    {
        dev_extend_add(p, fronts, f, 0, tm[2], 1);
        __threadfence_block();
        __syncthreads();
    }
    const bool direct = kids && p.ea_lds && p.ea_direct;
    const bool mirror_now = p.panel16 && (!kids || direct);
    if (direct)
    {
        const int e1 = DBG_DELAY(p) == 30 ? tm[16] : tm[17];
        if (mirror_now)
            dev_potrf_load_children<true>(p, fronts, fronts + foff, fld, ncs, tm[16], e1, Ls, dinv);
        else
            dev_potrf_load_children(p, fronts, fronts + foff, fld, ncs, tm[16], e1, Ls, dinv);
    }
    else if (mirror_now)
        dev_potrf_load<true>(fronts + foff, fld, ncs, Ls, dinv);
    else
        dev_potrf_load(fronts + foff, fld, ncs, Ls, dinv);
    stamp(0, 1);
    if (kids && p.ea_lds && !direct)
    {
        if (DBG_DELAY(p) != 30)
            dev_extend_add_lead(p, fronts, tm[16], tm[17], Ls, Vs + threadIdx.x);
    }
    if (p.panel16)
    {
        dev_potrf16(ncp, lds, p.winv + fwoff, fail, mirror_now, DBG_DELAY(p));
        stamp_value(0, 6, ncs);
        stamp(0, 7);
        kernel_release(p);
        return;
    }
    dev_potrf_panels(ncs, Ls, dinv, fail);
    __syncthreads();
    stamp(0, 5);
    {
        const int wv = __builtin_amdgcn_readfirstlane((int)(threadIdx.x >> 6));
        if (wv < (ncp >> 4))
            inv_diag16_wave(Ls, dinv, wv, Vs);
    }
    __syncthreads();
    dev_winv(Ls, ncp, Vs, p.winv + fwoff);
    stamp_value(0, 6, ncs);
    stamp(0, 7);
    kernel_release(p);
}

struct TileItem
{
    int a, b, ncs, nrs;
    long off, ld, woff, l21off;
};
__device__ __forceinline__ TileItem tile_item(const CholPlanDev& p, const int32_t* __restrict__ wl)
{
    const int32_t* ft = p.fat + 16 * ((int)((wl - p.wl_base) / 3) + (int)blockIdx.x);
    const long* f64 = reinterpret_cast<const long*>(ft + 8);
    return TileItem{ft[1], ft[2], ft[3], ft[4], f64[0], f64[1], f64[2], f64[3]};
}

__global__ __launch_bounds__(BIG) void k_up_trsyrk(CholPlanDev p, double* __restrict__ fronts,
                                                   const int32_t* __restrict__ wl)
{
#ifdef CUGO_DEBUG_HOOKS
    if (p.dbg_skip_wg == (int)blockIdx.x)
        return;
#endif
    kernel_acquire(p);
    extern __shared__ double lds[];
    dbg_fill_lds(p, lds);
    stamp(4, 0);
    const TileItem t = tile_item(p, wl);
    dev_trsyrk_tile<false>(fronts + t.off, t.ld, t.ncs, t.nrs + 1, t.nrs, t.a, t.b, p.winv + t.woff,
                           p.l21 + t.l21off, t.nrs + 1, lds, p.junk, 0);
    stamp(4, 7);
    stamp_value(4, 6, 1000000L * (t.a * 10 + t.b + 1) + 1000L * t.ncs + t.nrs);
    kernel_release(p);
}

__global__ __launch_bounds__(BIG) void k_up_trsyrk32(CholPlanDev p, double* __restrict__ fronts,
                                                     const int32_t* __restrict__ wl)
{
#ifdef CUGO_DEBUG_HOOKS
    if (p.dbg_skip_wg == (int)blockIdx.x)
        return;
#endif
    kernel_acquire(p);
    extern __shared__ double lds[];
    dbg_fill_lds(p, lds);
    const TileItem t = tile_item(p, wl);
    dev_trsyrk_tile32(fronts + t.off, t.ld, t.ncs, t.nrs + 1, t.nrs, t.a, t.b, p.winv + t.woff, p.l21 + t.l21off,
                      t.nrs + 1, lds, p.junk, 0);
    kernel_release(p);
}

__device__ __forceinline__ void dev_potrf_front(const CholPlanDev& p, double* __restrict__ fronts, int f,
                                                double* __restrict__ lds, int32_t* __restrict__ fail)
{
    const int ncs = 6 * p.ncb[f];
    const int ncp = pad16(ncs);
    double* Ls = lds;
    double* dinv = lds + NC_MAX * LLD;
    double* Vs = dinv + NC_MAX;
    dev_potrf_load(fronts + p.off[f], p.ldf[f], ncs, Ls, dinv);
    if (p.alias_of[f] < 0 && p.child_ptr[f + 1] > p.child_ptr[f])
    {
        dev_extend_add<true>(p, fronts, f, 0, p.ncb[f], 1, Ls, Vs + threadIdx.x);
        __syncthreads();
    }
    if (p.panel16)
    {
        dev_potrf16(ncp, lds, p.winv + p.woff[f], fail);
        return;
    }
    dev_potrf_panels(ncs, Ls, dinv, fail);
    __syncthreads();
    if ((int)(threadIdx.x >> 6) < (ncp >> 4))
        inv_diag16_wave(Ls, dinv, threadIdx.x >> 6, Vs);
    __syncthreads();
    dev_winv(Ls, ncp, Vs, p.winv + p.woff[f]);
}

__global__ __launch_bounds__(BIG) void k_up_potrf_la(CholPlanDev p, double* __restrict__ fronts,
                                                     int task0, int npotrf,
                                                     const int32_t* __restrict__ wl_tiles, int tile,
                                                     int32_t* __restrict__ fail)
{
    extern __shared__ double lds[];
    if ((int)blockIdx.x < npotrf)
    {
        dev_potrf_front(p, fronts, p.task_fronts[p.task_ptr[task0 + blockIdx.x]], lds, fail);
        return;
    }
    const int32_t* it = wl_tiles + 3 * (blockIdx.x - npotrf);
    const int f = it[0];
    const int ncs = 6 * p.ncb[f], nrs = 6 * (p.nb[f] - p.ncb[f]), q = 6 * p.la_np[f];
    if (tile == 32)
        dev_trsyrk_tile32(fronts + p.off[f], p.ldf[f], ncs, nrs + 1, nrs, it[1], it[2], p.winv + p.woff[f],
                          p.l21 + p.l21off[f], nrs + 1, lds, p.junk, q);
    else
        dev_trsyrk_tile<false>(fronts + p.off[f], p.ldf[f], ncs, nrs + 1, nrs, it[1], it[2],
                               p.winv + p.woff[f], p.l21 + p.l21off[f], nrs + 1, lds, p.junk, q);
}

__global__ __launch_bounds__(BIG) void k_up_lead(CholPlanDev p, double* __restrict__ fronts,
                                                 const int32_t* __restrict__ wl_lead, int nlead,
                                                 const int32_t* __restrict__ wl_eap, int neap,
                                                 const int32_t* __restrict__ wl_eab)
{
    extern __shared__ double lds[];
    if ((int)blockIdx.x >= nlead)
    {
        const int b = blockIdx.x - nlead;
        const int32_t* it = b < neap ? wl_eap + 3 * b : wl_eab + 3 * (b - neap);
        dev_extend_add(p, fronts, it[0], it[1], it[2], 4);
        return;
    }
    const int f = wl_lead[3 * blockIdx.x];
    const int ncb = p.ncb[f], np = p.la_np[f];
    const int ncs = 6 * ncb, nrs = 6 * (p.nb[f] - ncb), q = 6 * np;
    if (p.alias_of[f] < 0 && p.child_ptr[f + 1] > p.child_ptr[f])
    {
        dev_extend_add(p, fronts, f, 0, ncb + np, 3);
        __threadfence_block();
        __syncthreads();
    }
    dev_trsyrk_tile<true>(fronts + p.off[f], p.ldf[f], ncs, q, q, q > 64 ? 1 : 0, 0, p.winv + p.woff[f],
                          p.l21 + p.l21off[f], nrs + 1, lds, p.junk, 0);
}

constexpr int KC_SYRK2 = 48;
__global__ __launch_bounds__(BIG) void k_up_trsm(CholPlanDev p, double* __restrict__ fronts,
                                                 const int32_t* __restrict__ wl)
{
#ifdef CUGO_DEBUG_HOOKS
    if (p.dbg_skip_wg == (int)blockIdx.x)
        return;
#endif
    kernel_acquire(p);
    extern __shared__ double lds[];
    dbg_fill_lds(p, lds);
    const TileItem t = tile_item(p, wl);
    dev_trsm_w(fronts + t.off, t.ld, t.ncs, (long)t.ncs + t.a, t.b, p.winv + t.woff, lds, p.junk, p.l21 + t.l21off,
               t.nrs + 1);
    kernel_release(p);
}

__global__ __launch_bounds__(BIG) void k_up_syrk(CholPlanDev p, double* __restrict__ fronts,
                                                 const int32_t* __restrict__ wl)
{
#ifdef CUGO_DEBUG_HOOKS
    if (p.dbg_skip_wg == (int)blockIdx.x)
        return;
#endif
    kernel_acquire(p);
    extern __shared__ double lds[];
    dbg_fill_lds(p, lds);
    const TileItem t = tile_item(p, wl);
    dev_syrk_tiles<KC_SYRK2>(fronts + t.off, t.ld, t.ncs, t.nrs + 1, t.nrs, t.a, t.a + 1, t.b, lds, p.junk);
    kernel_release(p);
}

__device__ __forceinline__ void dev_backward_ahead(const CholPlanDev& p, const int32_t* __restrict__ ft, double* __restrict__ lds,
                                                   double* __restrict__ xnew)
{
    const int j0 = ft[1];
    const int ncs = ft[3], nrs = ft[4];
    const int r0 = 6 * ft[5];
    const double* L = p.l21 + reinterpret_cast<const long*>(ft + 8)[3];
    const long ldl = nrs + 1;
    const int c0 = ft[6];
    const int32_t* rows = p.rows + ft[7];
    double* xr = lds;
    for (int i = r0 + threadIdx.x; i < nrs; i += blockDim.x)
    {
        const int ib = i / 6;
        xr[i] = xnew[6L * rows[ib] + (i - 6 * ib)];
    }
    TILE_SYNC();
    const int j = j0 + (threadIdx.x >> 6), lane = threadIdx.x & 63;
    if (j < ncs)
    {
        const double* col = L + (long)j * ldl;
        const double y = col[nrs];
        double s = 0;
        for (int i = r0 + lane; i < nrs; i += 512)
        {
            double a[8];
#pragma unroll
            for (int u = 0; u < 8; u++)
                a[u] = col[min(i + 64 * u, nrs - 1)];
#pragma unroll
            for (int u = 0; u < 8; u++)
                s += (i + 64 * u < nrs) ? a[u] * xr[i + 64 * u] : 0.0;
        }
#pragma unroll
        for (int off = 32; off > 0; off >>= 1)
            s += __shfl_xor(s, off, 64);
        if (lane == 0)
            xnew[6L * c0 + j] = y - s;
    }
}

__global__ __launch_bounds__(BIG) void k_backward_stage(CholPlanDev p,
                                                        const double* __restrict__ fronts,
                                                        int task0, int ntasks,
                                                        const int32_t* __restrict__ wl_gemv,
                                                        double* __restrict__ xnew,
                                                        double* __restrict__ xout)
{
#ifdef CUGO_DEBUG_HOOKS
    if (p.dbg_skip_wg == (int)blockIdx.x)
        return;
#endif
    kernel_acquire(p);
    extern __shared__ double lds[];
    dbg_fill_lds(p, lds);
    if ((int)blockIdx.x >= ntasks)
    {
        dev_backward_ahead(p, p.fat + 16 * ((int)((wl_gemv - p.wl_base) / 3) + ((int)blockIdx.x - ntasks)), lds, xnew);
        kernel_release(p);
        return;
    }
    stamp(3, 0);
    const int task = task0 + blockIdx.x;
    const int32_t* tm = p.tmeta + cugo_k::TMETA * task;
    if (tm[0] == 1)
        dev_backward(p, fronts, front_view(tm), lds, xnew, xout, tm + 20);
    else
        for (int fi = p.task_ptr[task + 1] - 1; fi >= p.task_ptr[task]; fi--)
            dev_backward(p, fronts, front_view(p, p.task_fronts[fi]), lds, xnew, xout);
    stamp(3, 7);
    kernel_release(p);
}

typedef __attribute__((address_space(1))) unsigned int gu32;
typedef __attribute__((address_space(1))) unsigned long long gu64;
#ifdef CUGO_STAMPS
__device__ long long* g_bc_stamps = nullptr;
__device__ __forceinline__ void bc_stamp(int ticket, int slot)
{
    if (g_bc_stamps && threadIdx.x == 0)
        g_bc_stamps[3 * ticket + slot] = (long long)__builtin_amdgcn_s_memrealtime();
}
#else
__device__ __forceinline__ void bc_stamp(int, int) {}
#endif
constexpr unsigned long long BW_SPIN_TICKS = 25000000ULL;

__device__ __forceinline__ void bw_wait(gu32* word, unsigned epoch, gu32* st, int32_t* fail, unsigned* h_error)
{
    if (__hip_atomic_load(word, __ATOMIC_RELAXED, __HIP_MEMORY_SCOPE_AGENT) == epoch)
        return;
    const unsigned long long t0 = __builtin_amdgcn_s_memrealtime();
    for (;;)
    {
        __builtin_amdgcn_s_sleep(1);
        if (__hip_atomic_load(word, __ATOMIC_RELAXED, __HIP_MEMORY_SCOPE_AGENT) == epoch)
            return;
        if (__hip_atomic_load(st + cugo_k::BC_ABORT, __ATOMIC_RELAXED, __HIP_MEMORY_SCOPE_AGENT) != 0)
            return;
        if (__builtin_amdgcn_s_memrealtime() - t0 > BW_SPIN_TICKS)
        {
            __hip_atomic_store(st + cugo_k::BC_ABORT, 1u, __ATOMIC_RELAXED, __HIP_MEMORY_SCOPE_AGENT);
            __hip_atomic_store(st + cugo_k::BC_ERROR, 1u, __ATOMIC_RELAXED, __HIP_MEMORY_SCOPE_AGENT);
            __hip_atomic_store(fail, 1, __ATOMIC_RELAXED, __HIP_MEMORY_SCOPE_AGENT);
            __hip_atomic_store(h_error, 1u, __ATOMIC_RELAXED, __HIP_MEMORY_SCOPE_SYSTEM);
            return;
        }
    }
}

__global__ __launch_bounds__(BIG) void k_backward_chain(CholPlanDev p, const double* __restrict__ fronts,
                                                        double* xnew, double* __restrict__ xout, unsigned* state,
                                                        unsigned ticket_base, unsigned epoch, int32_t* fail,
                                                        unsigned* h_error)
{
    kernel_acquire(p);
    extern __shared__ double lds[];
    dbg_fill_lds(p, lds);
    gu32* st = (gu32*)state;
    double* vs = lds;
    int* tk = reinterpret_cast<int*>(lds + NC_MAX);
    if (threadIdx.x == 0)
        *tk = (int)(__hip_atomic_fetch_add(st + cugo_k::BC_HEAD, 1u, __ATOMIC_RELAXED, __HIP_MEMORY_SCOPE_AGENT) - ticket_base);
    __syncthreads();
    const int t = __builtin_amdgcn_readfirstlane(*tk);
    if (t < 0 || t >= (int)gridDim.x)
        return;
#ifdef CUGO_DEBUG_HOOKS
    const bool skip = p.dbg_skip_wg == t;
#else
    const bool skip = false;
#endif
    bc_stamp(t, 0);
    const int32_t* rc = p.bc_rec + cugo_k::BC_REC * t;
    const int f = rc[0], ncb = rc[1], nb = rc[2], c0 = rc[3], nseg = rc[6];
    const int32_t* rows = p.rows + rc[4];
    const int32_t* sg = p.bc_seg + 4 * rc[5];
    const long* r64 = reinterpret_cast<const long*>(rc + 8);
    const long l21o = r64[1], ld = r64[3];
    const int ncs = 6 * ncb, nrs = 6 * (nb - ncb), ncp = pad16(ncs);
    const double* L = l21o >= 0 ? p.l21 + l21o : fronts + r64[2] + ncs;
    const long ldl = l21o >= 0 ? nrs + 1 : ld;
    const double* Wg = p.winv + r64[0];
    const int g = threadIdx.x >> 3, l8 = threadIdx.x & 7;
    const bool colok = g < ncs;
    const int j = min(g, ncs - 1);
    const double* col = L + (long)j * ldl;
    const double* wcol = Wg + (long)j * ncp;
    const int jb = j / 6, comp = j - 6 * jb;
    double wv[12];
    const int k0 = (j & ~15) + 2 * l8;
#pragma unroll
    for (int u = 0; u < 6; u++)
    {
        const double2 v = *reinterpret_cast<const double2*>(wcol + min(k0 + 16 * u, ncp - 2));
        wv[2 * u] = v.x, wv[2 * u + 1] = v.y;
    }
    const double y = col[nrs];
    const int pj = p.perm[c0 + jb];
    for (int jj = ncs + threadIdx.x; jj < ncp; jj += blockDim.x)
        vs[jj] = 0.0;
    gu64* xg = (gu64*)xnew;
    double s = 0;
    for (int q = nseg - 1; q >= 0; q--)
    {
        const int a = sg[4 * q], rb = sg[4 * q + 1], n6 = 6 * sg[4 * q + 2];
        double b[12];
        int xi[6];
#pragma unroll
        for (int u = 0; u < 6; u++)
        {
            const int i = min(2 * l8 + 16 * u, n6 - 2);
            const double2 v = *reinterpret_cast<const double2*>(col + (6 * rb + i));
            b[2 * u] = v.x, b[2 * u + 1] = v.y;
            xi[u] = 6 * rows[rb + i / 6] + i % 6;
        }
#ifdef CUGO_DEBUG_HOOKS
        if (p.dbg_delay == 31 && (t & 1) && q == nseg - 1)
            dbg_sleep();
#endif
        if (threadIdx.x < 64)
            bw_wait(st + cugo_k::BC_DONE + a, epoch, st, fail, h_error);
        TILE_SYNC();
        if (q == 0)
            bc_stamp(t, 1);
        __builtin_amdgcn_fence(__ATOMIC_ACQUIRE, "wavefront");
        double x[12];
#pragma unroll
        for (int u = 0; u < 6; u++)
        {
            x[2 * u] = __longlong_as_double((long long)__hip_atomic_load(xg + xi[u], __ATOMIC_RELAXED, __HIP_MEMORY_SCOPE_AGENT));
            x[2 * u + 1] = __longlong_as_double((long long)__hip_atomic_load(xg + xi[u] + 1, __ATOMIC_RELAXED, __HIP_MEMORY_SCOPE_AGENT));
        }
#pragma unroll
        for (int u = 0; u < 12; u++)
            s += (2 * l8 + 16 * (u >> 1) < n6) ? b[u] * x[u] : 0.0;
    }
#pragma unroll
    for (int off = 4; off > 0; off >>= 1)
        s += __shfl_xor(s, off, 8);
    if (l8 == 0 && colok)
        vs[j] = y - s;
    TILE_SYNC();
    double xj = 0;
#pragma unroll
    for (int u = 0; u < 12; u++)
    {
        const int k = k0 + 16 * (u >> 1) + (u & 1);
        xj += (k < ncp) ? wv[u] * vs[k] : 0.0;
    }
#pragma unroll
    for (int off = 4; off > 0; off >>= 1)
        xj += __shfl_xor(xj, off, 8);
    if (l8 == 0 && colok && !skip)
    {
        __hip_atomic_store(xg + (6L * (c0 + jb) + comp), (unsigned long long)__double_as_longlong(xj), __ATOMIC_RELAXED,
                           __HIP_MEMORY_SCOPE_AGENT);
        xout[6L * pj + comp] = xj;
    }
    asm volatile("s_waitcnt vmcnt(0)" ::: "memory");
#ifdef CUGO_DEBUG_HOOKS
    if (p.dbg_delay == 31 && (t & 1))
        dbg_sleep();
#endif
    __syncthreads();
    bc_stamp(t, 2);
    if (threadIdx.x == 0)
        __hip_atomic_store(st + cugo_k::BC_DONE + f, epoch, __ATOMIC_RELAXED, __HIP_MEMORY_SCOPE_AGENT);
    kernel_release(p);
}

__global__ __launch_bounds__(CBS) void k_unpermute(CholPlanDev p, const double* __restrict__ xnew, double* __restrict__ xout)
{
    const int i = blockIdx.x * CBS + threadIdx.x;
    if (i < 6 * p.n)
        xout[6L * p.perm[i / 6] + i % 6] = xnew[i];
}

__global__ __launch_bounds__(CBS) void k_xs_pack(const int64_t* __restrict__ off, int B, int n,
                                                 const double* __restrict__ sys, double* __restrict__ xbuf)
{
    const long i = (long)blockIdx.x * CBS + threadIdx.x;
    const long nH = 36L * B;
    if (i >= nH + 6L * n)
        return;
    const long dst = i < nH ? off[i / 36] + i % 36 : off[B + (i - nH) / 6] + (i - nH) % 6;
    xbuf[dst] = sys[i];
}
__global__ __launch_bounds__(CBS) void k_xs_unpack(const int64_t* __restrict__ off, int B, int n,
                                                   const double* __restrict__ xbuf, double* __restrict__ sys,
                                                   long lo, long hi, long top0)
{
    const long i = (long)blockIdx.x * CBS + threadIdx.x;
    const long nH = 36L * B;
    if (i >= nH + 6L * n)
        return;
    const long o = i < nH ? off[i / 36] : off[B + (i - nH) / 6];
    if ((o >= lo && o < hi) || o >= top0)
        sys[i] = xbuf[o + (i < nH ? i % 36 : (i - nH) % 6)];
}

__global__ void k_flag_to_double(int32_t* __restrict__ flag)
{
    const int v = *flag;
    *reinterpret_cast<double*>(flag) = v ? 1.0 : 0.0;
}

#ifdef CUGO_DEBUG_HOOKS
struct DbgSkip
{
    int launch = 0, target_launch = -1, target_wg = -1;
    std::FILE* dump = nullptr;
};
static DbgSkip g_skip;
static inline CholPlanDev with_lds(const CholPlanDev& p, size_t lds_bytes, const char* name, int grid, int first = 0)
{
    CholPlanDev q = p;
    q.lds_doubles = (int)(lds_bytes / sizeof(double));
    q.dbg_skip_wg = -1;
    static int tile_delay_on_device = 0;
    if (p.dbg_delay != tile_delay_on_device)
    {
        (void)hipMemcpyToSymbol(HIP_SYMBOL(g_dbg_tile_delay), &p.dbg_delay, sizeof(int));
        tile_delay_on_device = p.dbg_delay;
    }
    if (g_skip.dump || g_skip.target_launch >= 0)
    {
        if (g_skip.dump)
            std::fprintf(g_skip.dump, "%d %s %d %d\n", g_skip.launch, name, grid, first);
        if (g_skip.launch == g_skip.target_launch)
            q.dbg_skip_wg = g_skip.target_wg;
        g_skip.launch++;
    }
    return q;
}
#else
static inline const CholPlanDev& with_lds(const CholPlanDev& p, size_t, const char*, int, int = 0) { return p; }
#endif
void ensure_lds(const void* fn, size_t bytes)
{
    if (bytes > 48 * 1024)
        (void)hipFuncSetAttribute(fn, hipFuncAttributeMaxDynamicSharedMemorySize, (int)bytes);
}

}

namespace cugo_k
{
#ifdef CUGO_DEBUG_HOOKS
void chol_dbg_skip_begin(int target_launch, int target_wg, const char* dump_path)
{
    if (g_skip.dump)
        std::fclose(g_skip.dump), g_skip.dump = nullptr;
    g_skip.launch = 0, g_skip.target_launch = target_launch, g_skip.target_wg = target_wg;
    if (dump_path)
        g_skip.dump = std::fopen(dump_path, "w");
}
void chol_dbg_skip_end()
{
    if (g_skip.dump)
        std::fclose(g_skip.dump), g_skip.dump = nullptr;
    g_skip.target_launch = -1;
}
#endif

size_t chol_lds_factor_bytes(int nc_max)
{
    (void)nc_max;
    const size_t trsm = (size_t)NC_MAX * LLD + NC_MAX + std::max((size_t)(NC_MAX >> 4) * (16 * 17), (size_t)NC_MAX * PSTB);
    const size_t syrk = (size_t)syrk_lds();
    return (std::max(trsm, syrk) + 8) * sizeof(double);
}
size_t chol_lds_potrf_bytes()
{
    return std::max((size_t)NC_MAX * LLD + NC_MAX + (NC_MAX >> 4) * (16 * 17) + 8, (size_t)p16::LDS_DOUBLES + 8) *
           sizeof(double);
}
int chol_max_pivot_cols() { return NC_MAX; }
size_t chol_lds_backward_bytes(int nc_max, long ld_max)
{
    const size_t ncp = (size_t)((nc_max + 15) & ~15);
    return (ncp + (size_t)ld_max + 8) * sizeof(double);
}

void set_debug_stamps(long long* d_buf)
{
#ifdef CUGO_STAMPS
    (void)hipMemcpyToSymbol(HIP_SYMBOL(g_stamps), &d_buf, sizeof(d_buf));
#else
    (void)d_buf;
#endif
}
void set_chain_stamps(long long* d_buf)
{
#ifdef CUGO_STAMPS
    (void)hipMemcpyToSymbol(HIP_SYMBOL(g_bc_stamps), &d_buf, sizeof(d_buf));
#else
    (void)d_buf;
#endif
}

void launch_chol_assemble(hipStream_t s, const CholPlanDev& p, double* d_fronts,
                          size_t front_doubles, const double* d_Hsc, double lambda,
                          const double* d_bsc, int32_t* d_fail, const int32_t* d_clear_items, int nclear,
                          const int32_t* d_asm_items, int nasm)
{
    if (d_asm_items && nasm > 0)
    {
        const long n = 36L * p.n_hsc_blocks;
        const int nblk = (int)((n + CBS - 1) / CBS), nrhs = std::max(1, (6 * p.n + CBS - 1) / CBS);
        CUGO_LAUNCH(k_assemble_fronts, dim3(nasm + nblk + nrhs), dim3(CBS), 0, s, p, d_fronts, d_Hsc, lambda, d_bsc,
                    d_fail, (int)((d_asm_items - p.wl_base) / 3), nasm, nblk);
        return;
    }
    if (nclear > 0)
        CUGO_LAUNCH(k_clear_fronts, dim3(nclear), dim3(CBS), 0, s, p, d_fronts, d_clear_items);
    else
        (void)hipMemsetAsync(d_fronts, 0, front_doubles * sizeof(double), s);
    const long n = 36L * p.n_hsc_blocks;
    const int nblk = (int)((n + CBS - 1) / CBS), nrhs = std::max(1, (6 * p.n + CBS - 1) / CBS);
    CUGO_LAUNCH(k_assemble_blocks, dim3(nblk + nrhs), dim3(CBS), 0, s, p, d_fronts, d_Hsc, lambda, d_bsc, d_fail,
                nblk);
}

void launch_chol_subtree_stage(hipStream_t s, const CholPlanDev& p, double* d_fronts, int task0,
                               int ntasks, size_t lds_bytes, int32_t* d_fail)
{
    if (ntasks <= 0)
        return;
    ensure_lds(reinterpret_cast<const void*>(k_subtree_factor), lds_bytes);
    CUGO_LAUNCH(k_subtree_factor, dim3(ntasks), dim3(BIG), lds_bytes, s, p, d_fronts, task0,
                       d_fail);
}

void launch_chol_two_phase(hipStream_t s, const CholPlanDev& p, double* d_fronts, const int32_t* d_trsm, int ntrsm,
                           const int32_t* d_syrk, int nsyrk)
{
    const size_t lds_t = (size_t)NC_MAX * PSTB * sizeof(double), lds_s = (size_t)2 * KC_SYRK2 * PST * sizeof(double);
    if (ntrsm > 0)
    {
        ensure_lds(reinterpret_cast<const void*>(k_up_trsm), lds_t);
        CUGO_LAUNCH(k_up_trsm, dim3(ntrsm), dim3(BIG), lds_t, s, with_lds(p, lds_t, "k_up_trsm", ntrsm), d_fronts, d_trsm);
    }
    if (nsyrk > 0)
    {
        ensure_lds(reinterpret_cast<const void*>(k_up_syrk), lds_s);
        CUGO_LAUNCH(k_up_syrk, dim3(nsyrk), dim3(BIG), lds_s, s, with_lds(p, lds_s, "k_up_syrk", nsyrk), d_fronts, d_syrk);
    }
}

void launch_chol_upper_stage(hipStream_t s, const CholPlanDev& p, double* d_fronts, int task0,
                             int ntasks, const int32_t* d_wl, int eap0, int neap, int ea0, int nea,
                             int sy0, int nsy, int tile, size_t lds_bytes, int32_t* d_fail, double* dbg_line,
                             double* dbg_scratch)
{
    (void)lds_bytes;
    if (ntasks <= 0)
        return;
    ensure_lds(reinterpret_cast<const void*>(k_up_potrf), chol_lds_potrf_bytes());
    CUGO_LAUNCH(k_up_potrf, dim3(ntasks + neap + nea), dim3(BIG), chol_lds_potrf_bytes(), s, with_lds(p, chol_lds_potrf_bytes(), "k_up_potrf", ntasks + neap + nea, ntasks), d_fronts,
                task0, ntasks, d_wl + 3L * eap0, neap, d_wl + 3L * ea0, d_fail);
#ifdef CUGO_DEBUG_HOOKS
    if (dbg_line)
        launch_swap16(s, dbg_line, dbg_scratch);
#else
    (void)dbg_line, (void)dbg_scratch;
#endif
    if (tile == 0)
        return;
    if (nsy > 0 && tile == 32)
    {
        const size_t lds32 = (2 * KC_SYRK * TPST32 + 21 * 256) * sizeof(double);
        ensure_lds(reinterpret_cast<const void*>(k_up_trsyrk32), lds32);
        CUGO_LAUNCH(k_up_trsyrk32, dim3(nsy), dim3(BIG), lds32, s, with_lds(p, lds32, "k_up_trsyrk32", nsy), d_fronts, d_wl + 3L * sy0);
    }
    else if (nsy > 0)
    {
        ensure_lds(reinterpret_cast<const void*>(k_up_trsyrk), trsyrk_lds() * sizeof(double));
        CUGO_LAUNCH(k_up_trsyrk, dim3(nsy), dim3(BIG), trsyrk_lds() * sizeof(double), s,
                    with_lds(p, trsyrk_lds() * sizeof(double), "k_up_trsyrk", nsy), d_fronts, d_wl + 3L * sy0);
    }
#ifdef CUGO_DEBUG_HOOKS
    if (dbg_line)
        launch_swap16(s, dbg_line, dbg_scratch);
#endif
}

void launch_chol_potrf_la(hipStream_t s, const CholPlanDev& p, double* d_fronts, int task0, int ntasks,
                          const int32_t* d_tiles, int ntiles, int tile, int32_t* d_fail)
{
    if (ntasks + ntiles <= 0)
        return;
    const size_t lds32 = (2 * KC_SYRK * TPST32 + 21 * 256) * sizeof(double);
    const size_t bytes = std::max(chol_lds_potrf_bytes(),
                                  ntiles > 0 ? (tile == 32 ? lds32 : trsyrk_lds() * sizeof(double)) : size_t(0));
    ensure_lds(reinterpret_cast<const void*>(k_up_potrf_la), std::max(chol_lds_potrf_bytes(), trsyrk_lds() * sizeof(double)));
    CUGO_LAUNCH(k_up_potrf_la, dim3(ntasks + ntiles), dim3(BIG), bytes, s, p, d_fronts, task0, ntasks,
                d_tiles, tile, d_fail);
}

void launch_chol_lead(hipStream_t s, const CholPlanDev& p, double* d_fronts, const int32_t* d_lead,
                      int nlead, const int32_t* d_eap, int neap, const int32_t* d_eab, int neab)
{
    if (nlead + neap + neab <= 0)
        return;
    ensure_lds(reinterpret_cast<const void*>(k_up_lead), trsyrk_lds() * sizeof(double));
    CUGO_LAUNCH(k_up_lead, dim3(nlead + neap + neab), dim3(BIG), trsyrk_lds() * sizeof(double), s, p,
                d_fronts, d_lead, nlead, d_eap, neap, d_eab);
}

#ifdef CUGO_DEBUG_HOOKS
__global__ __launch_bounds__(256) void k_hash_words(const unsigned long long* __restrict__ p, size_t n,
                                                    unsigned long long* __restrict__ out)
{
    unsigned long long h = 0;
    for (size_t i = (size_t)blockIdx.x * 256 + threadIdx.x; i < n; i += (size_t)gridDim.x * 256)
        h += p[i] * (2 * i + 1);
    atomicAdd(out, h);
}
__global__ void k_swap16(double* __restrict__ a, double* __restrict__ b)
{
    const double x = a[threadIdx.x], y = b[threadIdx.x];
    a[threadIdx.x] = y, b[threadIdx.x] = x;
}
void launch_swap16(hipStream_t s, double* line, double* scratch) { hipLaunchKernelGGL(k_swap16, dim3(1), dim3(16), 0, s, line, scratch); }
__global__ void k_nop() {}
void launch_nop(hipStream_t s) { hipLaunchKernelGGL(k_nop, dim3(1), dim3(64), 0, s); }
void launch_hash_words(hipStream_t s, const void* p, size_t n_words, unsigned long long* out)
{
    if (n_words == 0)
        return;
    const int nb = (int)std::min<size_t>(512, (n_words + 255) / 256);
    hipLaunchKernelGGL(k_hash_words, dim3(nb), dim3(256), 0, s, static_cast<const unsigned long long*>(p), n_words, out);
}
#endif
void launch_flag_to_double(hipStream_t s, int32_t* d_flag) { CUGO_LAUNCH(k_flag_to_double, dim3(1), dim3(1), 0, s, d_flag); }

void launch_xs_pack(hipStream_t s, const int64_t* d_off, int B, int n, const double* d_sys, double* d_xbuf)
{
    const long total = 36L * B + 6L * n;
    if (total > 0)
        CUGO_LAUNCH(k_xs_pack, dim3((unsigned)((total + CBS - 1) / CBS)), dim3(CBS), 0, s, d_off, B, n, d_sys, d_xbuf);
}
void launch_xs_unpack(hipStream_t s, const int64_t* d_off, int B, int n, const double* d_xbuf, double* d_sys, long lo,
                      long hi, long top0)
{
    const long total = 36L * B + 6L * n;
    if (total > 0)
        CUGO_LAUNCH(k_xs_unpack, dim3((unsigned)((total + CBS - 1) / CBS)), dim3(CBS), 0, s, d_off, B, n, d_xbuf, d_sys,
                    lo, hi, top0);
}

void launch_chol_unpermute(hipStream_t s, const CholPlanDev& p, const double* d_xnew, double* d_x)
{
    if (p.n > 0)
        CUGO_LAUNCH(k_unpermute, dim3((6 * p.n + CBS - 1) / CBS), dim3(CBS), 0, s, p, d_xnew, d_x);
}

void launch_chol_backward_stage(hipStream_t s, const CholPlanDev& p, double* d_fronts, int task0,
                                int ntasks, size_t lds_bytes, double* d_xnew, double* d_x,
                                const int32_t* d_wl_gemv, int ngemv)
{
    if (ntasks <= 0)
        return;
    ensure_lds(reinterpret_cast<const void*>(k_backward_stage), lds_bytes);
    CUGO_LAUNCH(k_backward_stage, dim3(ntasks + ngemv), dim3(BIG), lds_bytes, s, with_lds(p, lds_bytes, "k_backward_stage", ntasks + ngemv, ntasks), d_fronts, task0,
                       ntasks, d_wl_gemv, d_xnew, d_x);
}

void launch_chol_backward_chain(hipStream_t s, const CholPlanDev& p, double* d_fronts, int nfronts, double* d_xnew,
                                double* d_x, uint32_t* d_state, uint32_t ticket_base, uint32_t epoch, int32_t* d_fail,
                                uint32_t* h_error)
{
    if (nfronts <= 0)
        return;
    const size_t lds_bytes = 96 * 1024;
    ensure_lds(reinterpret_cast<const void*>(k_backward_chain), lds_bytes);
    CUGO_LAUNCH(k_backward_chain, dim3(nfronts), dim3(BIG), lds_bytes, s, with_lds(p, lds_bytes, "k_backward_chain", nfronts),
                d_fronts, d_xnew, d_x, d_state, ticket_base, epoch, d_fail, h_error);
}

}
```

### cuda-bundle-adjustment_amd/csrc/kernels/kernels.h

```cpp
#pragma once
#include <hip/hip_runtime.h>
#include <stddef.h>
#include <stdint.h>

#include "../../../include/cugo_hip.h"

namespace cugo_k
{

struct LaunchHook
{
    virtual void begin(const char* kernel, hipStream_t s) = 0;
    virtual void end(const char* kernel, hipStream_t s) = 0;
    virtual ~LaunchHook() {}
};
void set_launch_hook(LaunchHook* h);
LaunchHook* launch_hook();
struct LaunchScope
{
    const char* name;
    hipStream_t s;
    LaunchHook* h;
    LaunchScope(const char* n, hipStream_t st) : name(n), s(st), h(launch_hook())
    {
        if (h)
            h->begin(name, s);
    }
    ~LaunchScope()
    {
        if (h)
            h->end(name, s);
    }
};
#define CUGO_LAUNCH(kernel, grid, block, lds, stream, ...)                          \
    do                                                                              \
    {                                                                               \
        ::cugo_k::LaunchScope _scope(#kernel, stream);                              \
        hipLaunchKernelGGL(kernel, grid, block, lds, stream, __VA_ARGS__);          \
    } while (0)

struct ReduceScratch
{
    double* d_partials;
    size_t capacity;
};

void launch_errors(hipStream_t s, const cugo_edges& ev, const double* d_poses, const double* d_lms,
                   cugo_robust rk, ReduceScratch rs, double* d_chi);

void launch_build(hipStream_t s, const cugo_edges& ev, const double* d_poses, const double* d_lms,
                  cugo_robust rk, double* d_Hpp, double* d_bp, double* d_Hll, double* d_bl,
                  void* d_Hpl, ReduceScratch rs, double* d_chi, double fuse_lambda = -1.0,
                  double* d_invHll = nullptr, void* d_T = nullptr, double* d_lmrec = nullptr, bool skip_poses = false,
                  bool chi_behind_scale = false);

void launch_trial_tail_from_build(hipStream_t s, const cugo_edges& ev, ReduceScratch rs, int n_scale_partials,
                                  double* d_out, const double* d_flag, double* h_out, double seq, unsigned* d_done,
                                  const double* d_icp_chi = nullptr, int n_icp_chi = 0);

void launch_max_diagonal(hipStream_t s, const double* d_Hpp, int nP, const double* d_Hll, int nL,
                         ReduceScratch rs, double* d_out);

struct SchurRows
{
    const int32_t* d_pose_rec = nullptr;
    int max_row_nnz = 0;
    const int32_t* d_off_pi = nullptr;
    int mfma = 1;
    bool xcd = true;
    const double* d_lmrec = nullptr;
    const double* d_poses = nullptr;
    ReduceScratch rs{nullptr, 0};
    double* d_bp_out = nullptr;
};
void launch_list_pos(hipStream_t s, const cugo_edges& ev, int n_list, size_t M, const int32_t* d_off_ei,
                     int32_t* d_pose_pos, int32_t* d_off_pi);
void launch_pose_rec(hipStream_t s, const cugo_edges& ev, int n, int32_t* d_rec);
bool schur_rows_usable(const cugo_hsc_struct& hs, int max_row_nnz);
void launch_schur(hipStream_t s, const cugo_edges& ev, const cugo_hsc_struct& hs, double lambda,
                  int damp_hsc_diag, const double* d_Hpp, const double* d_bp, const double* d_Hll,
                  const double* d_bl, const void* d_Hpl, double* d_invHll, void* d_T,
                  double* d_bsc, double* d_Hsc, bool have_T = false, SchurRows rows = SchurRows());

int launch_backsubst_update(hipStream_t s, const cugo_edges& ev, double lambda, double lambda_pose,
                            const double* d_invHll, const double* d_bl, const double* d_bp,
                            const void* d_Hpl, const double* d_xp, double* d_xl,
                            const double* d_poses_in, const double* d_lms_in, double* d_poses_out,
                            double* d_lms_out, ReduceScratch rs, double* d_scale,
                            const double* d_lmrec = nullptr);
void launch_errors_tail(hipStream_t s, const cugo_edges& ev, const double* d_poses, const double* d_lms,
                        cugo_robust rk, ReduceScratch rs, int n_scale_partials, double* d_out,
                        const double* d_flag, double* h_out, double seq, unsigned* d_done,
                        const double* d_icp_chi = nullptr, int n_icp_chi = 0);

size_t reduce_scratch_doubles(int n_edges, int n_poses, int n_landmarks);

size_t icp_scratch_doubles(const cugo_icp_edges& ev);
int icp_check_indices(hipStream_t s, const cugo_icp_edges& ev, ReduceScratch rs);
void launch_icp_build(hipStream_t s, const cugo_icp_edges& ev, const double* d_poses, double* d_Hpp, double* d_bp,
                      ReduceScratch rs, double* d_chi, bool chi_add = false);
void launch_icp_errors(hipStream_t s, const cugo_icp_edges& ev, const double* d_poses, ReduceScratch rs, double* d_chi,
                       bool chi_add = false, double* d_edge_chi = nullptr);
void launch_icp_chunks(hipStream_t s, const cugo_icp_edges& ev, const double* d_poses, bool full, ReduceScratch rs,
                       double* d_edge_chi = nullptr);
void launch_icp_add(hipStream_t s, const cugo_icp_edges& ev, ReduceScratch rs, double* d_Hpp, double* d_bp);
void launch_icp_add_schur(hipStream_t s, const cugo_icp_edges& ev, ReduceScratch rs, const int32_t* d_rowptr,
                          double* d_Hsc, double* d_bp, double* d_bsc);
const double* icp_chunk_chi(const cugo_icp_edges& ev, ReduceScratch rs, int* n);
void launch_icp_chi_total(hipStream_t s, const cugo_icp_edges& ev, ReduceScratch rs, double* d_chi, bool chi_add);

void launch_edge_chi(hipStream_t s, const cugo_edges& e, const double* d_poses, const double* d_lms,
                     cugo_robust rk, double* d_chi_e);

constexpr int TMETA = 36;
constexpr int EA1_REC = 16;
struct CholPlanDev
{
    int n_fronts;
    const int32_t* ncb;
    const int32_t* nb;
    const int64_t* off;
    const int64_t* ldf;
    const int32_t* alias_of;
    const int32_t* bw_np;
    const int32_t* la_np;
    const int64_t* woff;
    double* winv;
    const int64_t* l21off;
    double* l21;
    int nc_max;
    int ea_lds;
    int panel16;
    int ea_direct;
#ifdef CUGO_DEBUG_HOOKS
    int kernel_acquire;
    int dbg_delay;
    int zero_lds;
    int lds_doubles;
    int dbg_skip_wg;
#endif
    const int32_t* col0;
    const int32_t* rows_ptr;
    const int32_t* rows;
    const int32_t* child_ptr;
    const int32_t* child;
    const int32_t* rel_ptr;
    const int32_t* rel;
    int n_stages;
    const int32_t* ea1;
    const int32_t* tmeta;
    const int32_t* asm_map;
    const int64_t* asm_off;
    const int32_t* wl_base;
    const int32_t* fat;
    const int32_t* bc_rec;
    const int32_t* bc_seg;
    const int32_t* task_ptr;
    const int32_t* task_fronts;
    int n_hsc_blocks;
    const int32_t* blk_front;
    const int32_t* blk_row;
    const int32_t* blk_col;
    const uint8_t* blk_trans;
    int n;
    const int32_t* perm;
    const int32_t* col_front;
    double* junk;
};

void launch_chol_assemble(hipStream_t s, const CholPlanDev& p, double* d_fronts, size_t front_doubles,
                          const double* d_Hsc, double lambda, const double* d_bsc, int32_t* d_fail,
                          const int32_t* d_clear_items, int nclear, const int32_t* d_asm_items = nullptr,
                          int nasm = 0);
void launch_chol_subtree_stage(hipStream_t s, const CholPlanDev& p, double* d_fronts, int task0,
                               int ntasks, size_t lds_bytes, int32_t* d_fail);
void launch_chol_upper_stage(hipStream_t s, const CholPlanDev& p, double* d_fronts, int task0,
                             int ntasks, const int32_t* d_wl, int eap0, int neap, int ea0, int nea,
                             int sy0, int nsy, int tile, size_t lds_bytes, int32_t* d_fail,
                             double* dbg_line = nullptr, double* dbg_scratch = nullptr);
#ifdef CUGO_DEBUG_HOOKS
void launch_swap16(hipStream_t s, double* line, double* scratch);
#endif
void launch_chol_two_phase(hipStream_t s, const CholPlanDev& p, double* d_fronts, const int32_t* d_trsm, int ntrsm,
                           const int32_t* d_syrk, int nsyrk);
void launch_chol_potrf_la(hipStream_t s, const CholPlanDev& p, double* d_fronts, int task0, int ntasks,
                          const int32_t* d_tiles, int ntiles, int tile, int32_t* d_fail);
void launch_chol_lead(hipStream_t s, const CholPlanDev& p, double* d_fronts, const int32_t* d_lead,
                      int nlead, const int32_t* d_eap, int neap, const int32_t* d_eab, int neab);
void launch_chol_backward_stage(hipStream_t s, const CholPlanDev& p, double* d_fronts, int task0,
                                int ntasks, size_t lds_bytes, double* d_xnew, double* d_x,
                                const int32_t* d_wl_gemv, int ngemv);
constexpr int BC_REC = 16, BC_HEAD = 0, BC_ABORT = 32, BC_ERROR = 33, BC_DONE = 64;
void launch_chol_backward_chain(hipStream_t s, const CholPlanDev& p, double* d_fronts, int nfronts, double* d_xnew,
                                double* d_x, uint32_t* d_state, uint32_t ticket_base, uint32_t epoch, int32_t* d_fail,
                                uint32_t* h_error);
#ifdef CUGO_DEBUG_HOOKS
void launch_nop(hipStream_t s);
void chol_dbg_skip_begin(int target_launch, int target_wg, const char* dump_path);
void chol_dbg_skip_end();
void launch_hash_words(hipStream_t s, const void* p, size_t n_words, unsigned long long* out);
#endif
void launch_flag_to_double(hipStream_t s, int32_t* d_flag);
void launch_chol_unpermute(hipStream_t s, const CholPlanDev& p, const double* d_xnew, double* d_x);
void launch_xs_pack(hipStream_t s, const int64_t* d_off, int B, int n, const double* d_sys, double* d_xbuf);
void launch_xs_unpack(hipStream_t s, const int64_t* d_off, int B, int n, const double* d_xbuf, double* d_sys, long lo,
                      long hi, long top0);
void set_debug_stamps(long long* d_buf);
void set_chain_stamps(long long* d_buf);
size_t chol_lds_factor_bytes(int nc_max);
size_t chol_lds_backward_bytes(int nc_max, long ld_max);
int chol_max_pivot_cols();

void launch_selinv_rows(hipStream_t s, const CholPlanDev& p, const double* d_fronts, double* d_sig,
                        const int64_t* d_sinfo, const int32_t* d_items, int nitems);
void launch_selinv_jj(hipStream_t s, const CholPlanDev& p, const double* d_fronts, double* d_sig, int task0,
                      int ntasks);
void launch_selinv_subtree(hipStream_t s, const CholPlanDev& p, const double* d_fronts, double* d_sig,
                           const int64_t* d_sinfo, int task0, int ntasks);
void launch_selinv_gather(hipStream_t s, const CholPlanDev& p, const double* d_sig, double* d_out);
int selinv_row_tile();
void launch_cov_pose_diag(hipStream_t s, int P, const int32_t* d_rowptr, const double* d_sigma, double* d_out);
void launch_lm_covariance(hipStream_t s, int L, const int32_t* d_lm_ptr, const int32_t* d_e_pose,
                          const uint8_t* d_flags, const double* d_Hll, const double* d_Hpl, const int32_t* d_rowptr,
                          const int32_t* d_colind, const double* d_sigma, double* d_out, int32_t* d_fail);

}
```

Before: 640.9 million.

## Group chained fronts in backward-chain kernel and skip root-only tile stages

The backward-substitution chain kernel now processes groups of up to two alias-chained supernodal fronts per workgroup. It reuses the child's boundary segments and passes solved values through LDS, so there is one global handoff and atomic wait per group instead of per front. The symbolic phase builds these groups and validates them. Separately, factor stages whose SYRK/TRSM items touch only root fronts skip those launches, and a flag in the chain record has the chain kernel compute that front's forward solve inline. This shortens the serial dependency chain and cuts launch counts, at the cost of more complex kernel code and more register pressure.

```diff
diff --git a/cuda-bundle-adjustment_amd/csrc/host/c_api.cpp b/cuda-bundle-adjustment_amd/csrc/host/c_api.cpp
--- a/cuda-bundle-adjustment_amd/csrc/host/c_api.cpp
+++ b/cuda-bundle-adjustment_amd/csrc/host/c_api.cpp
@@ -409,6 +409,8 @@
     CUGO_PLAN_FIELD(bc_front);
     CUGO_PLAN_FIELD(bc_seg_ptr);
     CUGO_PLAN_FIELD(bc_seg);
+    CUGO_PLAN_FIELD(bc_group_ptr);
+    CUGO_PLAN_FIELD(bc_group_front);
 #undef CUGO_PLAN_FIELD
     if (n == "asm_info")
     {
diff --git a/cuda-bundle-adjustment_amd/csrc/host/chol_solver.cpp b/cuda-bundle-adjustment_amd/csrc/host/chol_solver.cpp
--- a/cuda-bundle-adjustment_amd/csrc/host/chol_solver.cpp
+++ b/cuda-bundle-adjustment_amd/csrc/host/chol_solver.cpp
@@ -121,7 +121,48 @@
     }
     for (size_t k = 0; k < P.bc_seg.size() / 3; k++)
         std::memcpy(bc_seg.data() + 4 * k, P.bc_seg.data() + 3 * k, 3 * sizeof(int32_t));
-    const size_t o_bc_rec = put32(bc_rec), o_bc_seg = put32(bc_seg);
+    skip_tiles.assign(P.n_stages, 0);
+    for (int st = 0; st < P.n_stages && chain_form(); st++)
+    {
+        auto only_roots = [&](int i0, int i1) {
+            for (int i = i0; i < i1; i++)
+            {
+                const int f = P.wl[3 * i];
+                if (P.sparent[f] >= 0 || P.nb[f] != P.ncb[f])
+                    return false;
+            }
+            return true;
+        };
+        const bool two_phase = P.stage_tile[st] == 0;
+        const int n_items = P.syrk_ptr[st + 1] - P.syrk_ptr[st] + (two_phase ? P.trsm_ptr[st + 1] - P.trsm_ptr[st] : 0);
+        if (n_items == 0 || !only_roots(P.syrk_ptr[st], P.syrk_ptr[st + 1]) ||
+            (two_phase && !only_roots(P.trsm_ptr[st], P.trsm_ptr[st + 1])))
+            continue;
+        skip_tiles[st] = 1;
+        for (int t = P.stage_task_ptr[st]; t < P.stage_task_ptr[st + 1]; t++)
+            for (int fi = P.task_ptr[t]; fi < P.task_ptr[t + 1]; fi++)
+            {
+                const int f = P.task_fronts[fi];
+                if (P.sparent[f] < 0 && P.nb[f] == P.ncb[f])
+                    for (size_t tk = 0; tk < P.bc_front.size(); tk++)
+                        if (P.bc_front[tk] == f)
+                            bc_rec[cugo_k::BC_REC * tk + 7] = 1;
+            }
+    }
+    const size_t ngrp = P.bc_group_ptr.empty() ? 0 : P.bc_group_ptr.size() - 1;
+    std::vector<int32_t> bc_grp(cugo_k::BC_GRP * ngrp + 4, 0), ticket_of(P.n_super, -1);
+    for (size_t t = 0; t < P.bc_front.size(); t++)
+        ticket_of[P.bc_front[t]] = (int32_t)t;
+    for (size_t g = 0; g < ngrp; g++)
+    {
+        int32_t* m = bc_grp.data() + cugo_k::BC_GRP * g;
+        m[0] = P.bc_group_ptr[g + 1] - P.bc_group_ptr[g];
+        if (m[0] < 1 || m[0] > cugo_k::BC_GROUP_MAX)
+            throw std::runtime_error("cugo: a group of the backward chain is longer than the kernel takes");
+        for (int i = 0; i < m[0]; i++)
+            m[1 + i] = ticket_of[P.bc_group_front[P.bc_group_ptr[g] + i]];
+    }
+    const size_t o_bc_rec = put32(bc_rec), o_bc_seg = put32(bc_seg), o_bc_grp = put32(bc_grp);
     const size_t o_asm_map = put32(P.asm_map);
     const size_t o_trans = pack32.size();
     pack32.resize(o_trans + (P.blk_trans.size() + 3) / 4 + 4, 0);
@@ -131,7 +172,7 @@
     const size_t o_off = put64(P.off), o_woff = put64(P.woff), o_l21off = put64(P.l21off), o_ldf = put64(P.ldf);
     po = {o_ncb, o_nb, o_col0, o_alias, o_bwnp, o_lanp, o_rows_ptr, o_rows, o_child_ptr, o_child, o_rel_ptr, o_rel,
           o_task_ptr, o_task_fronts, o_blk_front, o_blk_row, o_blk_col, o_perm, o_col_front, o_wl, o_ea1, o_tmeta,
-          o_fat, o_asm_map, o_trans, o_asm_off, o_off, o_woff, o_l21off, o_ldf, o_bc_rec, o_bc_seg};
+          o_fat, o_asm_map, o_trans, o_asm_off, o_off, o_woff, o_l21off, o_ldf, o_bc_rec, o_bc_seg, o_bc_grp};
 }
 
 void cugo_chol::upload(hipStream_t s)
@@ -143,7 +184,7 @@
     const size_t o_blk_col = po[16], o_perm = po[17], o_col_front = po[18], o_wl = po[19], o_ea1 = po[20];
     const size_t o_tmeta = po[21], o_fat = po[22], o_asm_map = po[23], o_trans = po[24], o_asm_off = po[25];
     const size_t o_off = po[26], o_woff = po[27], o_l21off = po[28], o_ldf = po[29];
-    const size_t o_bc_rec = po[30], o_bc_seg = po[31];
+    const size_t o_bc_rec = po[30], o_bc_seg = po[31], o_bc_grp = po[32];
     d_pack32.upload(pack32, s), d_pack64.upload(pack64, s);
     d_fronts.resize((size_t)P.front_doubles + 16);
     d_fronts.zero(s);
@@ -151,7 +192,7 @@
     d_junk.resize(64 * 1024);
     d_winv.resize((size_t)P.winv_doubles + 16);
     d_l21.resize((size_t)P.l21_doubles + 16);
-    bw_chain = opt.bw_chain && !opt.lookahead && !P.has_subtree_stage && !P.bc_front.empty();
+    bw_chain = chain_form();
     if (bw_chain)
     {
         d_bc_state.resize((size_t)cugo_k::BC_DONE + P.n_super);
@@ -195,7 +236,7 @@
     d_wl_ptr = b32 + o_wl;
     D.wl_base = d_wl_ptr, D.fat = b32 + o_fat, D.ea1 = b32 + o_ea1;
     D.asm_map = b32 + o_asm_map, D.asm_off = b64 + o_asm_off;
-    D.bc_rec = b32 + o_bc_rec, D.bc_seg = b32 + o_bc_seg;
+    D.bc_rec = b32 + o_bc_rec, D.bc_seg = b32 + o_bc_seg, D.bc_grp = b32 + o_bc_grp;
     asm_fronts = opt.asm_fronts;
     lds_factor = cugo_k::chol_lds_factor_bytes(P.nc_max);
     lds_backward = cugo_k::chol_lds_backward_bytes(P.nc_max, P.ld_max);
@@ -211,6 +252,7 @@
 void cugo_chol::analyze_host(int n, const int32_t* rowptr, const int32_t* colind)
 {
     CholOptions copt = CholOptions::from_env();
+    copt.bw_group = opt.bw_group > 0 ? std::min(opt.bw_group, cugo_k::BC_GROUP_MAX) : cugo_k::BC_GROUP_DEFAULT;
     const bool own_forced = opt.own_subtrees == 1;
     if ((world > 1 || own_forced) && bcast && opt.own_subtrees != 0)
         copt.rank = rank, copt.world = world, copt.owned = true;
@@ -450,8 +492,9 @@
                 s, dev, d_fronts.data(), t0, t1 - t0, d_wl_ptr, plan.ea_ptr[st],
                 plan.ea_ptr[st + 1] - plan.ea_ptr[st], plan.eab_ptr[st],
                 plan.eab_ptr[st + 1] - plan.eab_ptr[st], plan.syrk_ptr[st],
-                plan.syrk_ptr[st + 1] - plan.syrk_ptr[st], plan.stage_tile[st], lds_factor, d_fail, stale, stale_scratch);
-            if (plan.stage_tile[st] == 0)
+                skip_tiles[st] ? 0 : plan.syrk_ptr[st + 1] - plan.syrk_ptr[st], plan.stage_tile[st], lds_factor, d_fail, stale,
+                stale_scratch);
+            if (plan.stage_tile[st] == 0 && !skip_tiles[st])
             {
                 cugo_k::launch_chol_two_phase(s, dev, d_fronts.data(), d_wl_ptr + 3L * plan.trsm_ptr[st],
                                               plan.trsm_ptr[st + 1] - plan.trsm_ptr[st],
@@ -483,12 +526,13 @@
     CUGO_HOOK(hooks.hash(14, d_fronts.data(), (size_t)plan.front_doubles));
     if (bw_chain)
     {
-        const int nf = (int)plan.bc_front.size();
+        const int nf = (int)plan.bc_front.size(), ng = (int)plan.bc_group_ptr.size() - 1;
         if (++bc_epoch == 0)
             bc_epoch = 1;
-        cugo_k::launch_chol_backward_chain(s, dev, d_fronts.data(), nf, d_xnew.data(), d_x, d_bc_state.data(), bc_base,
+        cugo_k::launch_chol_backward_chain(s, dev, d_fronts.data(), ng, d_xnew.data(), d_x, d_bc_state.data(), bc_base,
                                            bc_epoch, d_fail, h_bc_error.data());
-        bc_base += (uint32_t)nf;
+        bc_base += (uint32_t)ng;
+        (void)nf;
 #ifdef CUGO_STAMPS
         if (dbg)
         {
@@ -496,31 +540,36 @@
             static long long* d_cs = nullptr;
             if (++chain_calls == 4)
             {
-                CUGO_HIP(hipMalloc(reinterpret_cast<void**>(&d_cs), 3 * sizeof(long long) * (size_t)nf));
-                CUGO_HIP(hipMemset(d_cs, 0, 3 * sizeof(long long) * (size_t)nf));
+                CUGO_HIP(hipMalloc(reinterpret_cast<void**>(&d_cs), 4 * sizeof(long long) * (size_t)nf));
+                CUGO_HIP(hipMemset(d_cs, 0, 4 * sizeof(long long) * (size_t)nf));
                 cugo_k::set_chain_stamps(d_cs);
             }
             if (chain_calls == 5)
             {
-                std::vector<long long> h(3 * (size_t)nf);
-                std::vector<int> ticket(plan.n_super, -1);
+                std::vector<long long> h(4 * (size_t)nf);
+                std::vector<int> ticket(plan.n_super, -1), group(plan.n_super, -1);
                 for (int t = 0; t < nf; t++)
                     ticket[plan.bc_front[t]] = t;
+                for (int g = 0; g < ng; g++)
+                    for (int k = plan.bc_group_ptr[g]; k < plan.bc_group_ptr[g + 1]; k++)
+                        group[plan.bc_group_front[k]] = g;
                 CUGO_HIP(hipStreamSynchronize(s));
                 CUGO_HIP(hipMemcpy(h.data(), d_cs, h.size() * sizeof(long long), hipMemcpyDeviceToHost));
                 cugo_k::set_chain_stamps(nullptr);
                 long long first = h[0], last = 0;
                 for (int t = 0; t < nf; t++)
-                    first = std::min(first, h[3 * t]), last = std::max(last, h[3 * t + 2]);
-                std::printf("chain stamps: %d fronts, first start to last done %lld ticks (10 ns)\n", nf, last - first);
+                    first = std::min(first, h[4 * t]), last = std::max(last, h[4 * t + 3]);
+                std::printf("chain stamps: %d fronts in %d groups, first start to last done %lld ticks (10 ns)\n", nf, ng, last - first);
                 for (int f = plan.bc_front[nf - 1]; f >= 0; f = plan.sparent[f])
                 {
                     const int t = ticket[f], pa = plan.sparent[f];
-                    std::printf("  front %d ticket %d ncb %d rows %d: start +%lld", f, t, plan.ncb[f], plan.nb[f] - plan.ncb[f],
-                                h[3 * t] - first);
-                    if (pa >= 0)
-                        std::printf(" wait %lld work %lld", h[3 * t + 1] - h[3 * ticket[pa] + 2], h[3 * t + 2] - h[3 * t + 1]);
-                    std::printf(" done +%lld\n", h[3 * t + 2] - first);
+                    std::printf("  front %d ticket %d group %d ncb %d rows %d: start +%lld", f, t, group[f], plan.ncb[f],
+                                plan.nb[f] - plan.ncb[f], h[4 * t] - first);
+                    if (pa >= 0 && group[pa] == group[f])
+                        std::printf(" step %lld", h[4 * t + 2] - h[4 * ticket[pa] + 2]);
+                    else if (pa >= 0)
+                        std::printf(" wait %lld work %lld", h[4 * t + 1] - h[4 * ticket[pa] + 3], h[4 * t + 3] - h[4 * t + 1]);
+                    std::printf(" x +%lld done +%lld\n", h[4 * t + 2] - first, h[4 * t + 3] - first);
                 }
             }
         }
diff --git a/cuda-bundle-adjustment_amd/csrc/host/chol_solver.h b/cuda-bundle-adjustment_amd/csrc/host/chol_solver.h
--- a/cuda-bundle-adjustment_amd/csrc/host/chol_solver.h
+++ b/cuda-bundle-adjustment_amd/csrc/host/chol_solver.h
@@ -24,12 +24,14 @@
 
     std::vector<int32_t> pack32;
     std::vector<int64_t> pack64;
-    std::array<size_t, 32> po{};
+    std::array<size_t, 33> po{};
     cugo_host::DevBuf<int32_t> d_pack32;
     cugo_host::DevBuf<int64_t> d_pack64;
     const int32_t* d_wl_ptr = nullptr;
     cugo_host::DevBuf<double> d_fronts, d_xnew, d_junk, d_winv, d_l21;
     bool bw_chain = false;
+    bool chain_form() const { return opt.bw_chain && !opt.lookahead && !plan.has_subtree_stage && !plan.bc_front.empty(); }
+    std::vector<char> skip_tiles;
     cugo_host::DevBuf<uint32_t> d_bc_state;
     cugo_host::PinnedBuf<uint32_t> h_bc_error;
     uint32_t bc_base = 0, bc_epoch = 0;
diff --git a/cuda-bundle-adjustment_amd/csrc/host/chol_symbolic.cpp b/cuda-bundle-adjustment_amd/csrc/host/chol_symbolic.cpp
--- a/cuda-bundle-adjustment_amd/csrc/host/chol_symbolic.cpp
+++ b/cuda-bundle-adjustment_amd/csrc/host/chol_symbolic.cpp
@@ -1502,6 +1502,39 @@
         }
         P.bc_seg_ptr[f + 1] = (int32_t)(P.bc_seg.size() / 3);
     }
+    const int cap = std::max(1, opt.bw_group);
+    P.bc_group_ptr.assign(1, 0), P.bc_group_front.clear();
+    std::vector<int32_t> group_of(ns, -1);
+    for (int f : P.bc_front)
+    {
+        if (group_of[f] >= 0)
+            continue;
+        const int32_t g = (int32_t)P.bc_group_ptr.size() - 1;
+        int len = 0;
+        for (int c = f; c >= 0 && len < cap && ticket[c] >= 0 && group_of[c] < 0; c = P.alias_of[c], len++)
+        {
+            if (len > 0)
+            {
+                const int pa = P.bc_group_front.back();
+                const int s0 = P.bc_seg_ptr[c], s1 = P.bc_seg_ptr[c + 1], q0 = P.bc_seg_ptr[pa], q1 = P.bc_seg_ptr[pa + 1];
+                bool ok = P.sparent[c] == pa && s1 - s0 == q1 - q0 + 1 && P.bc_seg[3 * s0] == pa &&
+                          P.bc_seg[3 * s0 + 1] == 0 && P.bc_seg[3 * s0 + 2] == P.ncb[pa];
+                for (int k = 0; ok && k < q1 - q0; k++)
+                    ok = P.bc_seg[3 * (s0 + 1 + k)] == P.bc_seg[3 * (q0 + k)] &&
+                         P.bc_seg[3 * (s0 + 1 + k) + 1] == P.bc_seg[3 * (q0 + k) + 1] + P.ncb[pa] &&
+                         P.bc_seg[3 * (s0 + 1 + k) + 2] == P.bc_seg[3 * (q0 + k) + 2];
+                if (!ok)
+                    throw std::runtime_error("cugo: a front stored in its child's update block does not share the child's boundary segments");
+            }
+            group_of[c] = g;
+            P.bc_group_front.push_back(c);
+        }
+        P.bc_group_ptr.push_back((int32_t)P.bc_group_front.size());
+    }
+    for (int f : P.bc_front)
+        for (int k = P.bc_seg_ptr[f]; k < P.bc_seg_ptr[f + 1]; k++)
+            if (group_of[P.bc_seg[3 * k]] > group_of[f])
+                throw std::runtime_error("cugo: a boundary row of a front belongs to a group scheduled after its own");
     lap("9 backward chain");
 }
 
diff --git a/cuda-bundle-adjustment_amd/csrc/host/chol_symbolic.h b/cuda-bundle-adjustment_amd/csrc/host/chol_symbolic.h
--- a/cuda-bundle-adjustment_amd/csrc/host/chol_symbolic.h
+++ b/cuda-bundle-adjustment_amd/csrc/host/chol_symbolic.h
@@ -20,6 +20,7 @@
     int tile32_max_tiles = 64;
     int rank = 0, world = 1;
     bool owned = false;
+    int bw_group = 1;
     static CholOptions from_env();
 };
 
@@ -64,6 +65,7 @@
     std::vector<int32_t> trsm_ptr;
     std::vector<int32_t> bw_np;
     std::vector<int32_t> bc_front, bc_seg_ptr, bc_seg;
+    std::vector<int32_t> bc_group_ptr, bc_group_front;
     int nc_max = 6;
 
     std::vector<int32_t> owner;
diff --git a/cuda-bundle-adjustment_amd/csrc/host/options.h b/cuda-bundle-adjustment_amd/csrc/host/options.h
--- a/cuda-bundle-adjustment_amd/csrc/host/options.h
+++ b/cuda-bundle-adjustment_amd/csrc/host/options.h
@@ -27,6 +27,7 @@
     bool ea_lds = true, panel16 = true, asm_fronts = true;
     bool ea_direct = true;
     bool bw_chain = true;
+    int bw_group = 0;
     bool reduce_scatter = true;
 
     static Options from_env()
@@ -67,6 +68,8 @@
         o.ea_lds = !off("CUGO_EA_LDS"), o.panel16 = !off("CUGO_PANEL16"), o.asm_fronts = !off("CUGO_ASM_FRONTS");
         o.ea_direct = !off("CUGO_EA_DIRECT");
         o.bw_chain = !off("CUGO_BW_CHAIN");
+        if (const char* e = std::getenv("CUGO_BW_GROUP"))
+            o.bw_group = std::atoi(e) > 0 ? std::atoi(e) : 0;
         o.reduce_scatter = !off("CUGO_REDUCE_SCATTER");
         return o;
     }
diff --git a/cuda-bundle-adjustment_amd/csrc/kernels/chol_kernels.hip b/cuda-bundle-adjustment_amd/csrc/kernels/chol_kernels.hip
--- a/cuda-bundle-adjustment_amd/csrc/kernels/chol_kernels.hip
+++ b/cuda-bundle-adjustment_amd/csrc/kernels/chol_kernels.hip
@@ -2218,7 +2218,7 @@
 __device__ __forceinline__ void bc_stamp(int ticket, int slot)
 {
     if (g_bc_stamps && threadIdx.x == 0)
-        g_bc_stamps[3 * ticket + slot] = (long long)__builtin_amdgcn_s_memrealtime();
+        g_bc_stamps[4 * ticket + slot] = (long long)__builtin_amdgcn_s_memrealtime();
 }
 #else
 __device__ __forceinline__ void bc_stamp(int, int) {}
@@ -2248,6 +2248,34 @@
     }
 }
 
+constexpr int GM = cugo_k::BC_GROUP_MAX;
+
+__device__ __forceinline__ void bc_slice(double (&b)[12], const double* __restrict__ col, int row0, int l8, int n6)
+{
+#pragma unroll
+    for (int u = 0; u < 6; u++)
+    {
+        const int i = min(2 * l8 + 16 * u, n6 - 2);
+        const double2 v = *reinterpret_cast<const double2*>(col + (row0 + i));
+        b[2 * u] = v.x, b[2 * u + 1] = v.y;
+    }
+}
+__device__ __forceinline__ void bc_acc(double& s, const double (&b)[12], const double (&x)[12], int l8, int n6)
+{
+#pragma unroll
+    for (int u = 0; u < 12; u++)
+        s += (2 * l8 + 16 * (u >> 1) < n6) ? b[u] * x[u] : 0.0;
+}
+__device__ __forceinline__ void bc_wslice(double (&w)[12], const double* __restrict__ wcol, int k0, int ncp)
+{
+#pragma unroll
+    for (int u = 0; u < 6; u++)
+    {
+        const double2 v = *reinterpret_cast<const double2*>(wcol + min(k0 + 16 * u, ncp - 2));
+        w[2 * u] = v.x, w[2 * u + 1] = v.y;
+    }
+}
+
 __global__ __launch_bounds__(BIG) void k_backward_chain(CholPlanDev p, const double* __restrict__ fronts,
                                                         double* xnew, double* __restrict__ xout, unsigned* state,
                                                         unsigned ticket_base, unsigned epoch, int32_t* fail,
@@ -2258,114 +2286,232 @@
     dbg_fill_lds(p, lds);
     gu32* st = (gu32*)state;
     double* vs = lds;
-    int* tk = reinterpret_cast<int*>(lds + NC_MAX);
+    double* xs = lds + 2 * NC_MAX;
+    int* tk = reinterpret_cast<int*>(lds + 3 * NC_MAX);
     if (threadIdx.x == 0)
         *tk = (int)(__hip_atomic_fetch_add(st + cugo_k::BC_HEAD, 1u, __ATOMIC_RELAXED, __HIP_MEMORY_SCOPE_AGENT) - ticket_base);
     __syncthreads();
-    const int t = __builtin_amdgcn_readfirstlane(*tk);
-    if (t < 0 || t >= (int)gridDim.x)
-        return;
+    const int gt = __builtin_amdgcn_readfirstlane(*tk);
+    if (gt < 0 || gt >= (int)gridDim.x)
+        return;
+    const int32_t* gr = p.bc_grp + cugo_k::BC_GRP * gt;
+    const int m = min(gr[0], GM);
+    const int g = threadIdx.x >> 3, l8 = threadIdx.x & 7;
+    int tp[GM], fp[GM], ncs[GM], c0[GM], pj[GM];
+    int nrs_[GM];
+    long wo[GM];
+    const int32_t* sg[GM];
+    const double* col[GM];
+    double y[GM], s[GM];
+    gu64* xg = (gu64*)xnew;
+#pragma unroll
+    for (int i = 0; i < GM; i++)
+    {
+        tp[i] = gr[1 + min(i, m - 1)];
+        bc_stamp(tp[i], 0);
+        const int32_t* rc = p.bc_rec + cugo_k::BC_REC * tp[i];
+        fp[i] = rc[0], ncs[i] = 6 * rc[1], c0[i] = rc[3];
+        sg[i] = p.bc_seg + 4 * rc[5];
+        const long* r64 = reinterpret_cast<const long*>(rc + 8);
+        const long l21o = r64[1], ld = r64[3];
+        const int nrs = 6 * (rc[2] - rc[1]);
+        const double* L = l21o >= 0 ? p.l21 + l21o : fronts + r64[2] + ncs[i];
+        const long ldl = l21o >= 0 ? nrs + 1 : ld;
+        const int j = min(g, ncs[i] - 1);
+        col[i] = L + (long)j * ldl;
+        wo[i] = r64[0], nrs_[i] = nrs;
+        s[i] = 0;
+    }
+    auto ypj = [&](int i) __attribute__((always_inline)) {
+        y[i] = col[i][nrs_[i]];
+        pj[i] = p.perm[c0[i] + min(g, ncs[i] - 1) / 6];
+    };
+    ypj(0);
+    const int32_t* rows = p.rows + p.bc_rec[cugo_k::BC_REC * tp[0] + 4];
+    const int nseg = p.bc_rec[cugo_k::BC_REC * tp[0] + 6];
+    auto wslice = [&](double(&w)[12], int i) __attribute__((always_inline)) {
+        const int j = min(g, ncs[i] - 1), ncp = pad16(ncs[i]);
+        bc_wslice(w, p.winv + wo[i] + (long)j * ncp, (j & ~15) + 2 * l8, ncp);
+    };
+    double wv[12];
+    auto segment = [&](int q, bool last) __attribute__((always_inline)) {
+        const int a = sg[0][4 * q], rb = sg[0][4 * q + 1], n6 = 6 * sg[0][4 * q + 2];
+        double b[GM][12];
+        unsigned xi[6];
+#pragma unroll
+        for (int u = 0; u < 6; u++)
+        {
+            const int i = min(2 * l8 + 16 * u, n6 - 2);
+            xi[u] = 8u * (unsigned)(6 * rows[rb + i / 6] + i % 6);
+        }
+#pragma unroll
+        for (int i = 0; i < GM; i++)
+            if (i < m)
+                bc_slice(b[i], col[i], 6 * sg[i][4 * (q + i) + 1], l8, n6);
+        if (last)
+            wslice(wv, 0);
 #ifdef CUGO_DEBUG_HOOKS
-    const bool skip = p.dbg_skip_wg == t;
-#else
-    const bool skip = false;
-#endif
-    bc_stamp(t, 0);
-    const int32_t* rc = p.bc_rec + cugo_k::BC_REC * t;
-    const int f = rc[0], ncb = rc[1], nb = rc[2], c0 = rc[3], nseg = rc[6];
-    const int32_t* rows = p.rows + rc[4];
-    const int32_t* sg = p.bc_seg + 4 * rc[5];
-    const long* r64 = reinterpret_cast<const long*>(rc + 8);
-    const long l21o = r64[1], ld = r64[3];
-    const int ncs = 6 * ncb, nrs = 6 * (nb - ncb), ncp = pad16(ncs);
-    const double* L = l21o >= 0 ? p.l21 + l21o : fronts + r64[2] + ncs;
-    const long ldl = l21o >= 0 ? nrs + 1 : ld;
-    const double* Wg = p.winv + r64[0];
-    const int g = threadIdx.x >> 3, l8 = threadIdx.x & 7;
-    const bool colok = g < ncs;
-    const int j = min(g, ncs - 1);
-    const double* col = L + (long)j * ldl;
-    const double* wcol = Wg + (long)j * ncp;
-    const int jb = j / 6, comp = j - 6 * jb;
-    double wv[12];
-    const int k0 = (j & ~15) + 2 * l8;
-#pragma unroll
-    for (int u = 0; u < 6; u++)
-    {
-        const double2 v = *reinterpret_cast<const double2*>(wcol + min(k0 + 16 * u, ncp - 2));
-        wv[2 * u] = v.x, wv[2 * u + 1] = v.y;
-    }
-    const double y = col[nrs];
-    const int pj = p.perm[c0 + jb];
-    for (int jj = ncs + threadIdx.x; jj < ncp; jj += blockDim.x)
-        vs[jj] = 0.0;
-    gu64* xg = (gu64*)xnew;
-    double s = 0;
-    for (int q = nseg - 1; q >= 0; q--)
-    {
-        const int a = sg[4 * q], rb = sg[4 * q + 1], n6 = 6 * sg[4 * q + 2];
-        double b[12];
-        int xi[6];
-#pragma unroll
-        for (int u = 0; u < 6; u++)
-        {
-            const int i = min(2 * l8 + 16 * u, n6 - 2);
-            const double2 v = *reinterpret_cast<const double2*>(col + (6 * rb + i));
-            b[2 * u] = v.x, b[2 * u + 1] = v.y;
-            xi[u] = 6 * rows[rb + i / 6] + i % 6;
-        }
-#ifdef CUGO_DEBUG_HOOKS
-        if (p.dbg_delay == 31 && (t & 1) && q == nseg - 1)
+        if (p.dbg_delay == 31 && (gt & 1) && q == nseg - 1)
             dbg_sleep();
 #endif
         if (threadIdx.x < 64)
             bw_wait(st + cugo_k::BC_DONE + a, epoch, st, fail, h_error);
         TILE_SYNC();
-        if (q == 0)
-            bc_stamp(t, 1);
+        if (last)
+        {
+#pragma unroll
+            for (int i = 0; i < GM; i++)
+                bc_stamp(tp[i], 1);
+        }
         __builtin_amdgcn_fence(__ATOMIC_ACQUIRE, "wavefront");
         double x[12];
 #pragma unroll
         for (int u = 0; u < 6; u++)
         {
-            x[2 * u] = __longlong_as_double((long long)__hip_atomic_load(xg + xi[u], __ATOMIC_RELAXED, __HIP_MEMORY_SCOPE_AGENT));
-            x[2 * u + 1] = __longlong_as_double((long long)__hip_atomic_load(xg + xi[u] + 1, __ATOMIC_RELAXED, __HIP_MEMORY_SCOPE_AGENT));
-        }
-#pragma unroll
-        for (int u = 0; u < 12; u++)
-            s += (2 * l8 + 16 * (u >> 1) < n6) ? b[u] * x[u] : 0.0;
-    }
-#pragma unroll
-    for (int off = 4; off > 0; off >>= 1)
-        s += __shfl_xor(s, off, 8);
-    if (l8 == 0 && colok)
-        vs[j] = y - s;
-    TILE_SYNC();
-    double xj = 0;
-#pragma unroll
-    for (int u = 0; u < 12; u++)
-    {
-        const int k = k0 + 16 * (u >> 1) + (u & 1);
-        xj += (k < ncp) ? wv[u] * vs[k] : 0.0;
-    }
-#pragma unroll
-    for (int off = 4; off > 0; off >>= 1)
-        xj += __shfl_xor(xj, off, 8);
-    if (l8 == 0 && colok && !skip)
-    {
-        __hip_atomic_store(xg + (6L * (c0 + jb) + comp), (unsigned long long)__double_as_longlong(xj), __ATOMIC_RELAXED,
-                           __HIP_MEMORY_SCOPE_AGENT);
-        xout[6L * pj + comp] = xj;
-    }
+            gu64* xp = (gu64*)((__attribute__((address_space(1))) char*)xg + xi[u]);
+            x[2 * u] = __longlong_as_double((long long)__hip_atomic_load(xp, __ATOMIC_RELAXED, __HIP_MEMORY_SCOPE_AGENT));
+            x[2 * u + 1] = __longlong_as_double((long long)__hip_atomic_load(xp + 1, __ATOMIC_RELAXED, __HIP_MEMORY_SCOPE_AGENT));
+        }
+#pragma unroll
+        for (int i = 0; i < GM; i++)
+            if (i < m)
+                bc_acc(s[i], b[i], x, l8, n6);
+    };
+    for (int q = nseg - 1; q > 0; q--)
+        segment(q, false);
+    if (nseg > 0)
+        segment(0, true);
+    else
+    {
+        wslice(wv, 0);
+        const int32_t* rc0 = p.bc_rec + cugo_k::BC_REC * tp[0];
+        if (rc0[7])
+        {
+            const long* r64 = reinterpret_cast<const long*>(rc0 + 8);
+            const double* B = fronts + r64[2] + ncs[0];
+            const double* Wg = p.winv + r64[0];
+            const int nc = ncs[0], ncp = pad16(nc), j = min(g, nc - 1);
+            double* bs = lds + 4 * NC_MAX;
+            if ((int)threadIdx.x < ncp)
+                bs[threadIdx.x] = (int)threadIdx.x < nc ? B[(long)threadIdx.x * r64[3]] : 0.0;
+            double w[12];
+#pragma unroll
+            for (int u = 0; u < 6; u++)
+            {
+                const int k = min(2 * l8 + 16 * u, ncp - 2);
+                w[2 * u] = Wg[(long)k * ncp + j], w[2 * u + 1] = Wg[(long)(k + 1) * ncp + j];
+            }
+            TILE_SYNC();
+            double yj = 0;
+#pragma unroll
+            for (int u = 0; u < 12; u++)
+            {
+                const int k = 2 * l8 + 16 * (u >> 1) + (u & 1);
+                yj += (k <= (j | 15) && k < ncp) ? w[u] * bs[min(k, ncp - 1)] : 0.0;
+            }
+#pragma unroll
+            for (int off = 4; off > 0; off >>= 1)
+                yj += __shfl_xor(yj, off, 8);
+            y[0] = yj;
+        }
+    }
+    double bi[GM][12], wn[12];
+#pragma unroll
+    for (int i = 1; i < GM; i++)
+        if (i < m)
+        {
+            bc_slice(bi[i], col[i], 6 * sg[i][4 * (i - 1) + 1], l8, ncs[0]);
+            ypj(i);
+        }
+    if (1 < m)
+        wslice(wn, min(1, GM - 1));
+#pragma unroll
+    for (int pc = 0; pc < GM; pc++)
+        if (pc < m)
+        {
+            const int nc = ncs[pc], ncp = pad16(nc);
+            const bool colok = g < nc;
+            const int j = min(g, nc - 1), k0 = (j & ~15) + 2 * l8;
+#ifdef CUGO_DEBUG_HOOKS
+            const bool skip = p.dbg_skip_wg == tp[pc];
+#else
+            const bool skip = false;
+#endif
+            double sj = s[pc];
+#pragma unroll
+            for (int off = 4; off > 0; off >>= 1)
+                sj += __shfl_xor(sj, off, 8);
+            if (l8 == 0 && g < ncp)
+                vs[g] = colok ? y[pc] - sj : 0.0;
+            if (pc > 0)
+                asm volatile("s_waitcnt vmcnt(0)" ::: "memory");
+            TILE_SYNC();
+            if (pc > 0)
+            {
+                bc_stamp(tp[pc - 1], 3);
+                if (threadIdx.x == 0)
+                    __hip_atomic_store(st + cugo_k::BC_DONE + fp[pc - 1], epoch, __ATOMIC_RELAXED, __HIP_MEMORY_SCOPE_AGENT);
+            }
+            double xj = 0;
+#pragma unroll
+            for (int u = 0; u < 12; u++)
+            {
+                const int k = k0 + 16 * (u >> 1) + (u & 1);
+                xj += (k < ncp) ? wv[u] * vs[k] : 0.0;
+            }
+#pragma unroll
+            for (int off = 4; off > 0; off >>= 1)
+                xj += __shfl_xor(xj, off, 8);
+            if (l8 == 0 && colok)
+            {
+                gu64* xd = xg + (6L * c0[pc] + j);
+                if (!skip)
+                {
+                    __hip_atomic_store(xd, (unsigned long long)__double_as_longlong(xj), __ATOMIC_RELAXED, __HIP_MEMORY_SCOPE_AGENT);
+                    xout[6L * pj[pc] + (j % 6)] = xj;
+                }
+#ifdef CUGO_DEBUG_HOOKS
+                else
+                    xj = __longlong_as_double((long long)__hip_atomic_load(xd, __ATOMIC_RELAXED, __HIP_MEMORY_SCOPE_AGENT));
+#endif
+                xs[j] = xj;
+            }
+            if (pc + 1 < m)
+            {
+                TILE_SYNC();
+                bc_stamp(tp[pc], 2);
+                double x[12];
+#pragma unroll
+                for (int u = 0; u < 6; u++)
+                {
+                    const int i = min(2 * l8 + 16 * u, nc - 2);
+                    x[2 * u] = xs[i], x[2 * u + 1] = xs[i + 1];
+                }
+#pragma unroll
+                for (int i = pc + 1; i < GM; i++)
+                    if (i < m)
+                        bc_acc(s[i], bi[i], x, l8, nc);
+#pragma unroll
+                for (int i = pc + 2; i < GM; i++)
+                    if (i < m)
+                        bc_slice(bi[i], col[i], 6 * sg[i][4 * (i - 2 - pc) + 1], l8, ncs[min(pc + 1, GM - 1)]);
+#pragma unroll
+                for (int u = 0; u < 12; u++)
+                    wv[u] = wn[u];
+                if (pc + 2 < m)
+                    wslice(wn, min(pc + 2, GM - 1));
+            }
+        }
+    bc_stamp(tp[GM - 1], 2);
     asm volatile("s_waitcnt vmcnt(0)" ::: "memory");
 #ifdef CUGO_DEBUG_HOOKS
-    if (p.dbg_delay == 31 && (t & 1))
+    if (p.dbg_delay == 31 && (gt & 1))
         dbg_sleep();
 #endif
     __syncthreads();
-    bc_stamp(t, 2);
+    bc_stamp(tp[GM - 1], 3);
     if (threadIdx.x == 0)
-        __hip_atomic_store(st + cugo_k::BC_DONE + f, epoch, __ATOMIC_RELAXED, __HIP_MEMORY_SCOPE_AGENT);
+        __hip_atomic_store(st + cugo_k::BC_DONE + fp[GM - 1], epoch, __ATOMIC_RELAXED, __HIP_MEMORY_SCOPE_AGENT);
     kernel_release(p);
 }
 
@@ -2667,10 +2813,11 @@
                        ntasks, d_wl_gemv, d_xnew, d_x);
 }
 
-void launch_chol_backward_chain(hipStream_t s, const CholPlanDev& p, double* d_fronts, int nfronts, double* d_xnew,
+void launch_chol_backward_chain(hipStream_t s, const CholPlanDev& p, double* d_fronts, int ngroups, double* d_xnew,
                                 double* d_x, uint32_t* d_state, uint32_t ticket_base, uint32_t epoch, int32_t* d_fail,
                                 uint32_t* h_error)
 {
+    const int nfronts = ngroups;
     if (nfronts <= 0)
         return;
     const size_t lds_bytes = 96 * 1024;
diff --git a/cuda-bundle-adjustment_amd/csrc/kernels/kernels.h b/cuda-bundle-adjustment_amd/csrc/kernels/kernels.h
--- a/cuda-bundle-adjustment_amd/csrc/kernels/kernels.h
+++ b/cuda-bundle-adjustment_amd/csrc/kernels/kernels.h
@@ -155,6 +155,7 @@
     const int32_t* fat;
     const int32_t* bc_rec;
     const int32_t* bc_seg;
+    const int32_t* bc_grp;
     const int32_t* task_ptr;
     const int32_t* task_fronts;
     int n_hsc_blocks;
@@ -191,7 +192,9 @@
                                 int ntasks, size_t lds_bytes, double* d_xnew, double* d_x,
                                 const int32_t* d_wl_gemv, int ngemv);
 constexpr int BC_REC = 16, BC_HEAD = 0, BC_ABORT = 32, BC_ERROR = 33, BC_DONE = 64;
-void launch_chol_backward_chain(hipStream_t s, const CholPlanDev& p, double* d_fronts, int nfronts, double* d_xnew,
+constexpr int BC_GROUP_MAX = 2, BC_GROUP_DEFAULT = 2, BC_GRP = 8;
+static_assert(BC_GROUP_MAX >= 1 && BC_GROUP_MAX < BC_GRP && BC_GROUP_DEFAULT <= BC_GROUP_MAX, "a group record holds its pieces' tickets");
+void launch_chol_backward_chain(hipStream_t s, const CholPlanDev& p, double* d_fronts, int ngroups, double* d_xnew,
                                 double* d_x, uint32_t* d_state, uint32_t ticket_base, uint32_t epoch, int32_t* d_fail,
                                 uint32_t* h_error);
 #ifdef CUGO_DEBUG_HOOKS
```

Result: slower. 621.7 million (-3.0%).
